# talmolab/track-mjx

Hardware: AMD Instinct MI355X
Metric: env-steps/sec (whole node), rodent task @ 4096 envs/GPU (higher is better)
Workload: dtype f32

## Files before the change

include/tmjx.h:

```cpp
#ifndef TMJX_H
#define TMJX_H
#include <stddef.h>
#include <stdint.h>

#ifdef __cplusplus
extern "C" {
#endif

#define TMJX_OK 0
#define TMJX_EINVAL (-22)
#define TMJX_ENOMEM (-12)
#define TMJX_EHIP (-5)

typedef struct tmjx_model tmjx_model;

typedef struct tmjx_layout_t {
  int32_t nq, nv, nu, nbody, ncon, nefc, obs_size, ref_obs_size, n_metrics, window;
  int32_t qpos, qvel, act, qacc_warmstart, time;
  int32_t xpos, xmat_torso, qfrc_actuator;
  int32_t prev_ctrl, action_buffer, done, steps_f;
  int32_t first_phys, first_obs, first_prev_ctrl;
  int32_t state_rows;
  int32_t i_clip_idx, i_start_frame, i_buffer_index, i_nan_count, istate_rows;
  int32_t ws_rows;
} tmjx_layout_t;

int tmjx_model_create(const void *blob, size_t nbytes, tmjx_model **out);
void tmjx_model_destroy(tmjx_model *m);
int tmjx_layout(const tmjx_model *m, tmjx_layout_t *out);

int tmjx_set_wrappers(tmjx_model *m, int episode_length, int auto_reset);
int tmjx_set_action_repeat(tmjx_model *m, int action_repeat);

int tmjx_clips_upload(tmjx_model *m, const float *position, const float *quaternion, const float *joints,
                      const float *body_positions, const float *angular_velocity, int n_clips, int n_frames);

int tmjx_reset(tmjx_model *m, float *state, int32_t *istate, const int32_t *clip_idx, const int32_t *start_frame,
               const float *qpos_noise, const float *qvel_noise, float *obs, float *workspace, int n_env, void *stream);

int tmjx_step(tmjx_model *m, float *state, int32_t *istate, const float *action, float *obs, float *reward,
              float *done, float *truncation, float *metrics, float *workspace, int n_env, void *stream);

int tmjx_physics_step(tmjx_model *m, float *state, const float *action, float *workspace, int n_env, void *stream);

int tmjx_physics(tmjx_model *m, float *state, const float *action, int n_substeps, float *workspace, int n_env,
                 void *stream);
int tmjx_forward(tmjx_model *m, float *state, float *workspace, int n_env, void *stream);

int tmjx_reward_obs(tmjx_model *m, float *state, int32_t *istate, const float *action, float *obs, float *reward,
                    float *done, float *truncation, float *metrics, float *workspace, int n_env, void *stream);

int tmjx_reward_frame(tmjx_model *m, float *state, int32_t *istate, const float *action, const float *frame_pos,
                      const float *frame_quat, const float *frame_joints, const float *frame_bodypos, const float *frame_angvel,
                      float *obs, float *reward, float *done, float *truncation, float *metrics, int n_env, void *stream);

int tmjx_gae(const float *truncation, const float *termination, const float *rewards, const float *values,
             const float *bootstrap, float lambda_, float discount, float *vs, float *advantages, int T, int B,
             void *stream);

typedef struct {
  int32_t T, B, A, Z;
  float reward_scaling, discounting, gae_lambda, clip_eps, entropy_cost, kl_weight;
  int32_t normalize_advantage;
  int32_t accumulate;
} tmjx_ppo_cfg_t;
int tmjx_ppo_scratch_floats(int T, int B);
int tmjx_ppo_loss(const tmjx_ppo_cfg_t *cfg, const float *logits, const float *raw_action, const float *behaviour_logp,
                  const float *noise, const float *baseline, const float *bootstrap, const float *reward, const float *discount,
                  const float *truncation, const float *fc2, float *dlogits, float *dbaseline, float *dfc2, float *scratch,
                  float *out, void *stream);

#define TMJX_PPO_PHASE_A 1
#define TMJX_PPO_PHASE_B 2
#define TMJX_PPO_PHASE_C 4
#define TMJX_PPO_PHASE_D 8
int tmjx_ppo_loss_phases(const tmjx_ppo_cfg_t *cfg, const float *logits, const float *raw_action, const float *behaviour_logp,
                         const float *noise, const float *baseline, const float *bootstrap, const float *reward, const float *discount,
                         const float *truncation, const float *fc2, float *dlogits, float *dbaseline, float *dfc2, float *scratch,
                         float *out, int phases, void *stream);

int tmjx_silu_ln_partial_floats(int rows, int H);
int tmjx_silu_ln_fwd(const float *z, const float *bias, const float *gamma, const float *beta, float *y, float *stats, int rows, int H,
                     float eps, void *stream);
int tmjx_silu_ln_bwd(const float *dy, const float *z, const float *bias, const float *gamma, const float *stats, float *dz, float *grads,
                     float *partial, int rows, int H, void *stream);
int tmjx_silu_ln_fwd_bf16(const float *z, const float *bias, const float *gamma, const float *beta, uint16_t *y16, int ldy16, float *stats, int rows, int H,
                          float eps, void *stream);
int tmjx_silu_ln_bwd_bf16(const float *dy, const float *z, const float *bias, const float *gamma, const float *stats, uint16_t *dz16, int lddz16, float *grads,
                          float *partial, int rows, int H, void *stream);

int tmjx_gather_normalize(const float *src, const int64_t *idx, const float *mean, const float *std, float *out, int T, int R, int B,
                          int W, void *stream);
int tmjx_gather_minibatch(const float *obs, const float *next_last, const float *raw_action, const float *log_prob, const float *reward, const float *discount,
                          const float *truncation, const int64_t *idx, const float *mean, const float *std, float *obs_n, float *next_n, float *raw_action_g,
                          float *scalars_g, int T, int R, int B, int W, int A, void *stream);
#define TMJX_MINIBATCH_STATE_WORDS (16 + 16 * 64)
typedef struct tmjx_minibatch_t {
  const float *obs, *next_last, *raw_action, *log_prob, *reward, *discount, *truncation;
  const int64_t *perm;
  const float *mean, *std;
  float *obs_n, *next_n, *raw_action_g, *scalars_g;
  float *eps, *noise;
  int64_t *state;
  uint64_t seed;
  int32_t T, R, B, W, A, Z, advance;
} tmjx_minibatch_t;
int tmjx_minibatch_begin(const tmjx_minibatch_t *mb, void *stream);
int tmjx_minibatch_begin_bf16(const tmjx_minibatch_t *mb, uint16_t *obs_n16, int ld16, void *stream);
int tmjx_philox4x32_10(const uint32_t *ctr_key_dev, uint32_t *out_dev, void *stream);

int tmjx_latent_concat_bwd(const float *dx, const float *eps, const float *fc2, float *dfc2, int n, int Z, int dx_stride, void *stream);
int tmjx_latent_concat_bwd_add(const float *dx, const float *eps, const float *fc2, const float *add, float *dfc2, int n, int Z, int dx_stride,
                               void *stream);

int tmjx_latent_concat(const float *fc2, const float *eps, const float *obs, float *x, int n, int Z, int obs_w, int ref_w,
                       int64_t obs_s0, int64_t obs_s1, const float *mean, const float *std, int x_stride, uint64_t seed, const int64_t *rng_state,
                       void *stream);
int tmjx_sample_action(const float *logits, const float *noise, float *raw, float *action_t, float *logp, int n, int A, uint64_t seed,
                       int64_t *rng_state, void *stream);

int tmjx_linear_act_ok(const float *A, int64_t lda, const float *W, int ldw, int K);
int tmjx_linear_act(const float *A, int64_t lda, const float *W, int ldw, const float *bias, float *C, int M, int N, int K,
                    const float *mean, const float *inv_std, void *stream);
int tmjx_linear_nolds(const float *A, int64_t sa_row, int64_t sa_k, const float *W, const float *bias, float *C, int M, int N, int K,
                      void *stream);
int tmjx_linear_nolds_norm(const float *A, int64_t sa_row, int64_t sa_k, const float *W, const float *bias, float *C, int M, int N, int K,
                           const float *mean, const float *inv_std, void *stream);

int tmjx_linear_nolds_bf16(const float *A, int64_t sa_row, int64_t sa_k, const uint16_t *W, int ldw, const float *bias, float *C, int M, int N, int K,
                           const float *mean, const float *inv_std, void *stream);

int tmjx_colsum_scratch_floats(int width);
int tmjx_colsum(const float *src, float *out, float *scratch, int rows, int width, void *stream);

typedef struct tmjx_colsum_problem_t { const float *partial; float *out; int32_t rows, width; } tmjx_colsum_problem_t;
int tmjx_colsum_grouped(const tmjx_colsum_problem_t *problems, int n, void *stream);

int tmjx_adam_clip(float *param, const float *grad, float *exp_avg, float *exp_avg_sq, const float *grad_norm, long long n, float lr,
                   float beta1, float beta2, float eps, float bias_correction1, float bias_correction2, float max_norm, void *stream);
int tmjx_adam_norm_floats(void);
int tmjx_adam_clip_norm(float *param, const float *grad, float *exp_avg, float *exp_avg_sq, float *norm_scratch, float *norm_out, long long n, float lr,
                        float beta1, float beta2, float eps, float bias_correction1, float bias_correction2, float max_norm, void *stream);

int tmjx_gemm_nt(const float *A, int lda, const float *W, int ldw, const float *bias, float *C, int ldc, int M, int N, int K, void *stream);
int tmjx_gemm_nn(const float *A, int lda, const float *W, int ldw, float *C, int ldc, int M, int N, int K, void *stream);
int tmjx_gemm_nt_silu_ln_ok(const float *A, int lda, const float *W, int ldw, int N);
int tmjx_gemm_nt_silu_ln(const float *A, int lda, const float *W, int ldw, const float *bias, const float *gamma, const float *beta, float *Z, float *Y,
                         int ldc, float *stats, int M, int N, int K, float eps, void *stream);
int tmjx_gemm_nn_ln_bwd_ok(const float *dY, int ldy, const float *W, int ldw, int N);
long long tmjx_gemm_nn_ln_bwd_partial_floats(int M, int N);
int tmjx_gemm_nn_ln_bwd(const float *dY, int ldy, const float *W, int ldw, const float *z, const float *bias, const float *gamma, const float *stats,
                        float *dz, float *partial, int M, int N, int K, void *stream);
int tmjx_gemm_nt_silu_ok(const float *A, int lda, const float *W, int ldw);
int tmjx_gemm_nt_silu(const float *A, int lda, const float *W, int ldw, const float *bias, float *Z, float *Y, int ldc, int M, int N, int K, void *stream);
int tmjx_silu_fwd(const float *z, const float *bias, float *y, long long rows, int N, void *stream);
int tmjx_silu_bwd(const float *dy, const float *z, const float *bias, float *dz, long long rows, int N, void *stream);
int tmjx_gemm_nn_silu_bwd_ok(const float *dY, int ldy, const float *W, int ldw);
int tmjx_gemm_nn_silu_bwd(const float *dY, int ldy, const float *W, int ldw, const float *z, const float *bias, float *dZ, int M, int N, int K, void *stream);
int tmjx_silu_bwd_rank1(const float *dy1, const float *w1, const float *z, const float *bias, float *dz, long long rows, int N, void *stream);
long long tmjx_head_dw_scratch_floats(int M, int K);
int tmjx_head_dw(const float *dy1, const float *x, int ldx, float *dw, float *db, float *scratch, int M, int K, void *stream);
#define TMJX_CHAIN_MAX_HIDDEN 4
typedef struct { const float *W, *bias, *gamma, *beta; float *z, *y, *stats; int32_t K, ldw; } tmjx_chain_layer_t;
typedef struct {
  const float *A; int32_t lda, M, n_hidden, epi;
  tmjx_chain_layer_t hidden[TMJX_CHAIN_MAX_HIDDEN];
  const float *Wf, *bf; float *outf; int32_t Nf, ldwf, ldof;
  float eps;
  int32_t rows_alloc;
  const float *lat_eps; float *lat_out; const float *prop; int32_t lat_Z, lat_ld, prop_w, prop_ld;
  void *prof;
} tmjx_chain_fwd_t;
int tmjx_chain_rows(int M);
int tmjx_chain_fwd_ok(const tmjx_chain_fwd_t *chain);
int tmjx_chain_fwd(const tmjx_chain_fwd_t *chain, void *stream);
typedef struct { const float *W; int32_t ldw; const float *z, *bias, *gamma, *stats; float *dz, *partial; } tmjx_chain_bwd_stage_t;
typedef struct {
  const float *G; int32_t ldg, Kg, M, n_stages, epi;
  tmjx_chain_bwd_stage_t stage[TMJX_CHAIN_MAX_HIDDEN];
  const float *W0; int32_t ldw0, dx_cols; float *dx; int32_t lddx;
  int32_t rows_alloc;
  void *prof;
} tmjx_chain_bwd_t;
int tmjx_chain_bwd_ok(const tmjx_chain_bwd_t *chain);
int tmjx_chain_bwd(const tmjx_chain_bwd_t *chain, void *stream);

int tmjx_head_fwd_ok(const float *x, int ldx, const float *w, int K);
int tmjx_head_fwd(const float *x, int ldx, const float *w, const float *bias, float *y, int M, int K, void *stream);
long long tmjx_gemm_dw_scratch_floats(int M, int N, int K);
int tmjx_gemm_dw(const float *dY, int ldy, const float *X, int ldx, float *dW, float *db, float *scratch, int M, int N, int K, void *stream);
typedef struct tmjx_dw_problem_t {
  const float *dY, *X;
  float *dW, *db, *scratch;
  int32_t ldy, ldx, lddw, M, N, K;
} tmjx_dw_problem_t;
int tmjx_gemm_dw_grouped(const tmjx_dw_problem_t *problems, int n, void *stream);
int tmjx_gemm_dw_grouped_wgs(const tmjx_dw_problem_t *probs, int n, int target_wgs, void *stream);

typedef struct tmjx_bf16_shadow_t {
  const float *src;
  uint16_t *dst, *dst_t;
  int32_t N, K, ld_src, ld_dst, ld_dst_t;
} tmjx_bf16_shadow_t;
int tmjx_bf16_shadow(const tmjx_bf16_shadow_t *items, int n, void *stream);
int tmjx_bgemm_nt(const void *A, int a_is_f32, int lda, const uint16_t *B, int ldb, const float *bias, float *C, int ldc, int M, int N, int K,
                  void *stream);
int tmjx_bgemm_row_tile_ok(int N);
int tmjx_bf16_z_bytes(void);
long long tmjx_bgemm_partial_floats(int M, int N, int sums);
int tmjx_bgemm_ln_fwd(const void *A, int a_is_f32, int lda, const uint16_t *B, int ldb, const float *bias, const float *gamma, const float *beta, uint16_t *Z16, int ldz,
                      uint16_t *Y16, int ldy16, float *stats, int M, int N, int K, float eps, void *stream);
int tmjx_bgemm_ln_bwd(const void *dY, int dy_is_f32, int ldy, const uint16_t *Bt, int ldb, const uint16_t *z16, int ldz, const float *bias, const float *gamma,
                      const float *stats, uint16_t *dZ16, int lddz, float *partial, int M, int N, int K, void *stream);
int tmjx_bgemm_silu_fwd(const void *A, int a_is_f32, int lda, const uint16_t *B, int ldb, const float *bias, uint16_t *Z16, int ldz, uint16_t *Y16, int ldy16,
                        float *Yf, int ldyf, int M, int N, int K, void *stream);
int tmjx_bgemm_silu_bwd(const void *dY, int dy_is_f32, int ldy, const uint16_t *Bt, int ldb, const uint16_t *z16, int ldz, const float *bias, uint16_t *dZ16, int lddz,
                        float *partial, int M, int N, int K, void *stream);
int tmjx_bf_silu_bwd(const float *dY, int ldy, const uint16_t *z16, int ldz, const float *bias, uint16_t *dZ16, int lddz, float *partial, int M, int N, void *stream);
int tmjx_bf_silu_bwd_rank1(const float *dy1, const float *w1, const uint16_t *z16, int ldz, const float *bias, uint16_t *dZ16, int lddz, float *partial, int M, int N,
                           void *stream);
long long tmjx_bgemm_dw_scratch_floats(int M, int N, int K);
int tmjx_bgemm_dw(const void *dY, int y_is_f32, int ldy, const void *X, int x_is_f32, int ldx, float *dW, int lddw, float *db, float *scratch,
                  int M, int N, int K, void *stream);
typedef struct tmjx_bdw_problem_t {
  const void *dY, *X;
  float *dW, *db, *scratch;
  int32_t y_is_f32, x_is_f32, ldy, ldx, lddw, M, N, K;
} tmjx_bdw_problem_t;
int tmjx_bgemm_dw_grouped(const tmjx_bdw_problem_t *problems, int n, int target_wgs, void *stream);

typedef struct tmjx_rollout_store_t {
  const float *obs; float *obs_dst0, *obs_dst1;
  const float *raw; float *raw_dst;
  const float *logp; float *logp_dst;
  const float *reward; float *reward_dst;
  const float *done; float *discount_dst;
  const float *trunc; float *trunc_dst;
  int32_t n, W, A;
  float *obs_dst2;
} tmjx_rollout_store_t;
int tmjx_rollout_store(const tmjx_rollout_store_t *s, void *stream);
int tmjx_clips_share(tmjx_model *m, const tmjx_model *owner);

int tmjx_stats_scratch_floats(int W);
int tmjx_stats_sums(const float *src, const float *mean, float *sums, float *scratch, long long rows, int W, void *stream);
int tmjx_stats_apply(const float *sums, float n_added, float *count, float *mean, float *summed_variance, float *std, int W, float std_min,
                     float std_max, void *stream);

int tmjx_debug_rows(const tmjx_model *m, const char *name, int *row0, int *count);

const char *tmjx_last_error(void);
const char *tmjx_version(void);

#ifdef __cplusplus
}
#endif
#endif
```

track_mjx_amd/agent/networks.py:

```python
from __future__ import annotations

import math
import os
from typing import Sequence

import torch
import torch.nn as nn
import torch.nn.functional as F


def _lecun_uniform_(w: torch.Tensor) -> None:
    fan_in = w.shape[1]
    lim = math.sqrt(3.0 / fan_in)
    with torch.no_grad():
        w.uniform_(-lim, lim)


def _lecun_normal_(w: torch.Tensor) -> None:
    fan_in = w.shape[1]
    std = math.sqrt(1.0 / fan_in) / 0.87962566103423978
    with torch.no_grad():
        nn.init.trunc_normal_(w, mean=0.0, std=std, a=-2 * std, b=2 * std)


class gemm_inputs:
    dtype = None
    shadows = None
    twins = None

    def __init__(self, dtype, shadows=None, twins=None):
        self.new = (dtype, shadows if dtype is not None else None, twins if dtype is not None else None)

    def __enter__(self):
        self.old = (gemm_inputs.dtype, gemm_inputs.shadows, gemm_inputs.twins)
        gemm_inputs.dtype, gemm_inputs.shadows, gemm_inputs.twins = self.new

    def __exit__(self, *a):
        gemm_inputs.dtype, gemm_inputs.shadows, gemm_inputs.twins = self.old
        return False

    @staticmethod
    def twin_of(x2: torch.Tensor, K: int):
        tw = gemm_inputs.twins
        if not tw or x2.dtype != torch.float32:
            return None
        hit = tw.get(x2.data_ptr())
        if hit is None:
            return None
        t16, width = hit
        Ke = _ceil64(K)
        if t16.shape[0] != x2.shape[0] or x2.stride(0) != width or K > width or Ke > t16.shape[1] or os.environ.get("TMJX_NO_BF16_TWIN"):
            return None
        return t16[:, :Ke]


def _hip_gemm_ok(*ts) -> bool:
    return gemm_inputs.dtype is None and all(t.is_cuda and t.dtype == torch.float32 for t in ts)


def _rows2d(x: torch.Tensor) -> torch.Tensor:
    x2 = x.reshape(-1, x.shape[-1])
    return x2 if x2.stride(1) == 1 and (x2.shape[0] == 1 or x2.stride(0) >= x2.shape[1]) else x2.contiguous()


def _launch(fn_name: str, dev, *args):
    import ctypes as C
    from .. import hip as _hip
    L = _hip.lib()
    with torch.cuda.device(dev):
        _hip.check(getattr(L, fn_name)(*args, C.c_void_p(torch.cuda.current_stream(dev).cuda_stream)), fn_name)


def _p(t):
    import ctypes as C
    return C.c_void_p(t.data_ptr()) if t is not None else None


def gemm_nt(x: torch.Tensor, w: torch.Tensor, bias: torch.Tensor | None = None) -> torch.Tensor:
    x = _rows2d(x)
    w = w if w.stride(1) == 1 else w.contiguous()
    M, K = x.shape
    N = w.shape[0]
    y = torch.empty((M, N), dtype=torch.float32, device=x.device)
    if N == 1 and _head_kernels() and K % 4 == 0 and x.data_ptr() % 16 == 0 and x.stride(0) % 4 == 0 and w.data_ptr() % 16 == 0:
        _launch("tmjx_head_fwd", x.device, _p(x), x.stride(0), _p(w), _p(bias), _p(y), M, K)
        return y
    _launch("tmjx_gemm_nt", x.device, _p(x), x.stride(0), _p(w), w.stride(0), _p(bias), _p(y), N, M, N, K)
    return y


def _head_kernels() -> bool:
    return os.environ.get("TMJX_HEAD_KERNELS", "1") != "0"


def gemm_nn(dy: torch.Tensor, w: torch.Tensor, cols: int | None = None) -> torch.Tensor:
    dy = _rows2d(dy)
    w = w if w.stride(1) == 1 else w.contiguous()
    M, N = dy.shape
    K = w.shape[1]
    dx = torch.empty((M, K), dtype=torch.float32, device=dy.device)
    _launch("tmjx_gemm_nn", dy.device, _p(dy), dy.stride(0), _p(w), w.stride(0), _p(dx), K, M, K if cols is None else int(cols), N)
    return dx


def gemm_dw(dy: torch.Tensor, x: torch.Tensor, with_bias: bool):
    from .. import hip as _hip
    dy, x = _rows2d(dy), _rows2d(x)
    M, N = dy.shape
    K = x.shape[1]
    dw = torch.empty((N, K), dtype=torch.float32, device=dy.device)
    db = torch.empty(N, dtype=torch.float32, device=dy.device) if with_bias else None
    if N == 1 and _head_kernels() and dy.stride(0) == 1:
        scratch = torch.empty(int(_hip.lib().tmjx_head_dw_scratch_floats(M, K)), dtype=torch.float32, device=dy.device)
        _launch("tmjx_head_dw", dy.device, _p(dy), _p(x), x.stride(0), _p(dw), _p(db), _p(scratch), M, K)
        return dw, db
    scratch = torch.empty(int(_hip.lib().tmjx_gemm_dw_scratch_floats(M, N, K)), dtype=torch.float32, device=dy.device)
    _launch("tmjx_gemm_dw", dy.device, _p(dy), dy.stride(0), _p(x), x.stride(0), _p(dw), _p(db), _p(scratch), M, N, K)
    return dw, db


def _ceil64(n: int) -> int:
    return (int(n) + 63) // 64 * 64


def _ld(x2: torch.Tensor) -> int:
    return x2.stride(0) if x2.shape[0] > 1 else (x2.shape[1] + 7) // 8 * 8


def bgemm_nt(x: torch.Tensor, wb: torch.Tensor, N: int, K: int, bias: torch.Tensor | None = None, out: torch.Tensor | None = None) -> torch.Tensor:
    x = _rows2d(x)
    M = x.shape[0]
    y = torch.empty((M, N), dtype=torch.float32, device=x.device) if out is None else out
    _launch("tmjx_bgemm_nt", x.device, _p(x), int(x.dtype == torch.float32), _ld(x), _p(wb), wb.stride(0), _p(bias), _p(y), max(y.stride(0), N), M, N, K)
    return y


def bgemm_dw(dy: torch.Tensor, x: torch.Tensor, with_bias: bool, out: torch.Tensor | None = None, out_bias: torch.Tensor | None = None):
    from .. import hip as _hip
    dy, x = _rows2d(dy), _rows2d(x)
    M, N = dy.shape
    K = x.shape[1]
    dw = torch.empty((N, K), dtype=torch.float32, device=dy.device) if out is None else out
    db = (torch.empty(N, dtype=torch.float32, device=dy.device) if out_bias is None else out_bias) if with_bias else None
    d = deferred_weight_grads.active
    if d is not None and d.group_bf16 and N > 1 and out is not None:
        d.bproblems.append((dy, x, dw, db))
        return dw, db
    scratch = torch.empty(int(_hip.lib().tmjx_bgemm_dw_scratch_floats(M, N, K)), dtype=torch.float32, device=dy.device)
    _launch("tmjx_bgemm_dw", dy.device, _p(dy), int(dy.dtype == torch.float32), _ld(dy), _p(x), int(x.dtype == torch.float32), _ld(x),
            _p(dw), dw.stride(0) if N > 1 else max(dw.stride(0), K), _p(db), _p(scratch), M, N, K)
    return dw, db


def bf16_z_dtype() -> torch.dtype:
    from .. import hip as _hip
    return torch.float32 if int(_hip.lib().tmjx_bf16_z_bytes()) == 4 else torch.bfloat16


def bgemm_ln_fwd(x, wb, N: int, K: int, bias, gamma, beta, eps: float):
    x = _rows2d(x)
    M = x.shape[0]
    z = torch.empty((M, N), dtype=bf16_z_dtype(), device=x.device)
    y = torch.empty((M, N), dtype=torch.bfloat16, device=x.device)
    stats = torch.empty((M, 2), dtype=torch.float32, device=x.device)
    _launch("tmjx_bgemm_ln_fwd", x.device, _p(x), int(x.dtype == torch.float32), _ld(x), _p(wb), wb.stride(0), _p(bias), _p(gamma), _p(beta), _p(z), N, _p(y), N,
            _p(stats), M, N, K, float(eps))
    return z, y, stats


def bgemm_ln_bwd(dy, wtb, N: int, K: int, z, bias, gamma, stats):
    from .. import hip as _hip
    dy = _rows2d(dy)
    M = dy.shape[0]
    dz = torch.empty((M, N), dtype=torch.bfloat16, device=dy.device)
    partial = torch.empty(int(_hip.lib().tmjx_bgemm_partial_floats(M, N, 3)), dtype=torch.float32, device=dy.device)
    _launch("tmjx_bgemm_ln_bwd", dy.device, _p(dy), int(dy.dtype == torch.float32), _ld(dy), _p(wtb), wtb.stride(0), _p(z), z.stride(0), _p(bias), _p(gamma), _p(stats),
            _p(dz), N, _p(partial), M, N, K)
    return dz, partial.view(-1, 3, N)


def bgemm_silu_fwd(x, wb, N: int, K: int, bias, y_f32: bool = False):
    x = _rows2d(x)
    M = x.shape[0]
    ld = (N + 7) // 8 * 8
    z = torch.empty((M, ld), dtype=bf16_z_dtype(), device=x.device)[:, :N]
    y = torch.empty((M, ld), dtype=torch.float32 if y_f32 else torch.bfloat16, device=x.device)
    _launch("tmjx_bgemm_silu_fwd", x.device, _p(x), int(x.dtype == torch.float32), _ld(x), _p(wb), wb.stride(0), _p(bias), _p(z), ld,
            None if y_f32 else _p(y), ld, _p(y) if y_f32 else None, ld, M, N, K)
    return z, y[:, :N]


def bgemm_silu_bwd(dy, wtb, N: int, K: int, z, bias):
    from .. import hip as _hip
    dy = _rows2d(dy)
    M = dy.shape[0]
    ld = (N + 7) // 8 * 8
    dz = torch.empty((M, ld), dtype=torch.bfloat16, device=dy.device)
    partial = torch.empty(int(_hip.lib().tmjx_bgemm_partial_floats(M, N, 1)), dtype=torch.float32, device=dy.device)
    _launch("tmjx_bgemm_silu_bwd", dy.device, _p(dy), int(dy.dtype == torch.float32), _ld(dy), _p(wtb), wtb.stride(0), _p(z), z.stride(0), _p(bias), _p(dz), ld,
            _p(partial), M, N, K)
    return dz[:, :N], partial.view(-1, N)


class Bf16Shadows:

    def __init__(self, linears, need_t=None):
        from .. import hip as _hip
        self.lins = list(linears)
        need_t = set(self.lins if need_t is None else need_t)
        dev = self.lins[0].weight.device
        self.w, self.wt = {}, {}
        items = []
        for lin in self.lins:
            N, K = lin.weight.shape
            self.w[lin] = torch.zeros((N, _ceil64(K)), dtype=torch.bfloat16, device=dev)
            if lin in need_t:
                self.wt[lin] = torch.zeros((K, _ceil64(N)), dtype=torch.bfloat16, device=dev)
            t = self.wt.get(lin)
            items.append(_hip.Bf16Shadow(lin.weight.data_ptr(), self.w[lin].data_ptr(), t.data_ptr() if t is not None else None, N, K, lin.weight.stride(0),
                                         self.w[lin].stride(0), t.stride(0) if t is not None else 0))
        self._chunks = [(_hip.Bf16Shadow * len(items[i:i + 24]))(*items[i:i + 24]) for i in range(0, len(items), 24)]
        self._ptrs = [lin.weight.data_ptr() for lin in self.lins]

    def refresh(self) -> None:
        if self._ptrs != [lin.weight.data_ptr() for lin in self.lins]:
            raise RuntimeError("a parameter moved after its bf16 shadow was built (build the shadows after the flat optimiser re-seats the parameters)")
        dev = self.lins[0].weight.device
        for arr in self._chunks:
            _launch("tmjx_bf16_shadow", dev, arr, len(arr))


def _bf16_ok(x, lin) -> bool:
    sh = gemm_inputs.shadows
    return (gemm_inputs.dtype == torch.bfloat16 and sh is not None and lin in sh.w and x.is_cuda and x.dtype == torch.float32
            and lin.out_features % 4 == 0)


def _colsum(dy: torch.Tensor) -> torch.Tensor:
    if not (dy.is_cuda and dy.dtype == torch.float32 and dy.dim() == 2 and dy.is_contiguous() and dy.shape[0] >= 1024):
        return dy.sum(0)
    import ctypes as C
    from .. import hip as _hip
    L = _hip.lib()
    rows, width = dy.shape
    out = torch.empty(width, dtype=torch.float32, device=dy.device)
    scratch = torch.empty(L.tmjx_colsum_scratch_floats(width), dtype=torch.float32, device=dy.device)
    with torch.cuda.device(dy.device):
        _hip.check(L.tmjx_colsum(C.c_void_p(dy.data_ptr()), C.c_void_p(out.data_ptr()), C.c_void_p(scratch.data_ptr()), rows, width,
                                 C.c_void_p(torch.cuda.current_stream(dy.device).cuda_stream)), "tmjx_colsum")
    return out


class deferred_weight_grads:
    active = None

    def __enter__(self):
        self.problems, self.keep, self.colsums = [], [], []
        self.bproblems, self.group_bf16 = [], os.environ.get("TMJX_BDW_GROUPED", "1") != "0"
        self.seen: set = set()
        deferred_weight_grads.active = self
        return self

    def __exit__(self, *a):
        deferred_weight_grads.active = None
        return False

    @staticmethod
    def _aligned(t):
        return t.data_ptr() % 16 == 0 and t.stride(0) % 4 == 0 and t.stride(1) == 1

    def try_add(self, dy2, x2, w, b):
        gw, gb = w.grad, (b.grad if b is not None else None)
        if gw is None or (b is not None and gb is None) or len(self.problems) >= 16:
            return None
        if not (self._aligned(dy2) and self._aligned(x2) and gw.stride(1) == 1 and gw.shape == w.shape):
            return None
        if id(w) in self.seen:
            mine = [q for q in self.problems if q[2].data_ptr() == gw.data_ptr()]
            self.problems = [q for q in self.problems if q[2].data_ptr() != gw.data_ptr()]
            self._launch_problems(mine)
            return None
        self.seen.add(id(w))
        self.problems.append((dy2, x2, gw, gb))
        return gw, gb

    def launch_subset(self, pick, target_wgs: int = 0):
        mine = [q for q in self.problems if pick(q[2])]
        self.problems = [q for q in self.problems if not pick(q[2])]
        self._launch_problems(mine, target_wgs)

    def launch(self):
        import ctypes as C
        from .. import hip as _hip
        L = _hip.lib()
        if self.colsums:
            dev = self.colsums[0][0].device
            arr = (_hip.ColsumProblem * len(self.colsums))(*[_hip.ColsumProblem(pt.data_ptr(), g.data_ptr(), nb, wd) for pt, g, nb, wd in self.colsums])
            with torch.cuda.device(dev):
                _hip.check(L.tmjx_colsum_grouped(arr, len(self.colsums), C.c_void_p(torch.cuda.current_stream(dev).cuda_stream)), "tmjx_colsum_grouped")
            self.keep += [t for c in self.colsums for t in c[:2]]
            self.colsums = []
        self._launch_problems(self.problems)
        self.problems = []
        self._launch_bproblems()

    def _launch_bproblems(self):
        import ctypes as C
        from .. import hip as _hip
        probs, self.bproblems = self.bproblems, []
        if not probs:
            return
        L = _hip.lib()
        dev = probs[0][0].device
        for at in range(0, len(probs), 24):
            grp = probs[at:at + 24]
            sizes = [int(L.tmjx_bgemm_dw_scratch_floats(dy.shape[0], dy.shape[1], x.shape[1])) for dy, x, _, _ in grp]
            scratch = torch.empty(sum((n + 3) // 4 * 4 for n in sizes), dtype=torch.float32, device=dev)
            arr = (_hip.BdwProblem * len(grp))()
            off = 0
            for i, (dy, x, dw, db) in enumerate(grp):
                N, K = dy.shape[1], x.shape[1]
                arr[i] = _hip.BdwProblem(dy.data_ptr(), x.data_ptr(), dw.data_ptr(), db.data_ptr() if db is not None else None, scratch.data_ptr() + 4 * off,
                                         int(dy.dtype == torch.float32), int(x.dtype == torch.float32), _ld(dy), _ld(x), dw.stride(0) if N > 1 else max(dw.stride(0), K),
                                         dy.shape[0], N, K)
                off += (sizes[i] + 3) // 4 * 4
            with torch.cuda.device(dev):
                _hip.check(L.tmjx_bgemm_dw_grouped(arr, len(grp), 0, C.c_void_p(torch.cuda.current_stream(dev).cuda_stream)), "tmjx_bgemm_dw_grouped")
            self.keep += [scratch] + [t for q in grp for t in q[:2]]

    def _launch_problems(self, problems, target_wgs: int = 0):
        import ctypes as C
        from .. import hip as _hip
        if not problems:
            return
        L = _hip.lib()
        dev = problems[0][0].device
        sizes = [int(L.tmjx_gemm_dw_scratch_floats(dy.shape[0], dy.shape[1], x.shape[1])) for dy, x, _, _ in problems]
        scratch = torch.empty(sum((n + 3) // 4 * 4 for n in sizes), dtype=torch.float32, device=dev)
        arr = (_hip.DwProblem * len(problems))()
        off = 0
        for i, (dy, x, gw, gb) in enumerate(problems):
            arr[i] = _hip.DwProblem(dy.data_ptr(), x.data_ptr(), gw.data_ptr(), gb.data_ptr() if gb is not None else None,
                                    scratch.data_ptr() + 4 * off, dy.stride(0), x.stride(0), gw.stride(0), dy.shape[0], dy.shape[1], x.shape[1])
            off += (sizes[i] + 3) // 4 * 4
        with torch.cuda.device(dev):
            _hip.check(L.tmjx_gemm_dw_grouped_wgs(arr, len(problems), int(target_wgs), C.c_void_p(torch.cuda.current_stream(dev).cuda_stream)), "tmjx_gemm_dw_grouped")
        self.keep += [scratch] + [t for q in problems for t in q[:2]]


def chain_fwd_desc(x2, hidden, final=None, kind="ln", eps=1e-6, out=None, latent=None):
    from .. import hip as _hip
    M, dev = x2.shape[0], x2.device
    d = _hip.ChainFwd()
    d.A, d.lda, d.M, d.n_hidden, d.epi, d.eps = x2.data_ptr(), x2.stride(0), M, len(hidden), 1 if kind == "ln" else 3, float(eps)
    saved = []
    d.rows_alloc = rows = int(_hip.lib().tmjx_chain_rows(M))
    for l, h in enumerate(hidden):
        w, b = h[0], h[1]
        z = torch.empty((M, 256), dtype=torch.float32, device=dev)
        y = torch.empty((rows, 256), dtype=torch.float32, device=dev)[:M]
        st = torch.empty((M, 2), dtype=torch.float32, device=dev) if kind == "ln" else None
        L = d.hidden[l]
        L.W, L.bias, L.z, L.y, L.K, L.ldw = w.data_ptr(), b.data_ptr(), z.data_ptr(), y.data_ptr(), w.shape[1], w.stride(0)
        if kind == "ln":
            L.gamma, L.beta, L.stats = h[2].data_ptr(), h[3].data_ptr(), st.data_ptr()
        saved.append((z, y, st))
    if final is not None:
        wf, bf = final
        Nf = wf.shape[0]
        if out is None:
            out = torch.empty((M,) if Nf == 1 else (M, Nf), dtype=torch.float32, device=dev)
        d.Wf, d.bf, d.outf, d.Nf, d.ldwf, d.ldof = wf.data_ptr(), (bf.data_ptr() if bf is not None else None), out.data_ptr(), Nf, wf.stride(0), (1 if Nf == 1 else out.stride(0))
    if latent is not None:
        leps, dec_in, prop = latent
        d.lat_eps, d.lat_out, d.prop = leps.data_ptr(), dec_in.data_ptr(), prop.data_ptr()
        d.lat_Z, d.lat_ld, d.prop_w, d.prop_ld = leps.shape[1], dec_in.stride(0), prop.shape[1], prop.stride(0)
    return d, saved, out


def chain_fwd(x2, hidden, final=None, kind="ln", eps=1e-6, latent=None):
    import ctypes as C
    d, saved, out = chain_fwd_desc(x2, hidden, final, kind, eps, latent=latent)
    _launch("tmjx_chain_fwd", x2.device, C.byref(d))
    return saved, out


def chain_fwd_ok(x2, hidden, final=None, kind="ln") -> bool:
    import ctypes as C
    from .. import hip as _hip
    if os.environ.get("TMJX_NO_CHAIN") or not (x2.is_cuda and x2.dtype == torch.float32 and x2.dim() == 2 and x2.stride(1) == 1):
        return False
    if any(h[0].shape[0] != 256 for h in hidden) or not (1 <= len(hidden) <= 4):
        return False
    return bool(_hip.lib().tmjx_chain_fwd_ok(C.byref(chain_fwd_desc(x2[:1], hidden, final, kind)[0])))


def chain_bwd(g, final_w, blocks, kind="ln", w0=None, dx_cols=None, prof=None, dx_ld=None):
    import ctypes as C
    from .. import hip as _hip
    L = _hip.lib()
    M, dev = g.shape[0], g.device
    d = _hip.ChainBwd()
    head = g.dim() == 1
    d.G, d.ldg, d.Kg, d.M, d.n_stages, d.epi = g.data_ptr(), (1 if head else g.stride(0)), (1 if head else g.shape[1]), M, len(blocks), 2 if kind == "ln" else 4
    dzs, partials = [], []
    nfl = int(L.tmjx_gemm_nn_ln_bwd_partial_floats(M, 256)) if kind == "ln" else 0
    d.rows_alloc = rows = int(L.tmjx_chain_rows(M))
    for i, blk in enumerate(blocks):
        S = d.stage[i]
        w = final_w if i == 0 else blocks[i - 1][0]
        S.W, S.ldw = w.data_ptr(), (w.stride(0) if w.dim() == 2 and w.shape[0] > 1 else 256)
        dz = torch.empty((rows, 256), dtype=torch.float32, device=dev)[:M]
        S.z, S.bias, S.dz = blk[1].data_ptr(), blk[2].data_ptr(), dz.data_ptr()
        if kind == "ln":
            pt = torch.empty(nfl, dtype=torch.float32, device=dev)
            S.gamma, S.stats, S.partial = blk[3].data_ptr(), blk[4].data_ptr(), pt.data_ptr()
            partials.append(pt)
        dzs.append(dz)
    dx = None
    if w0 is not None:
        cols = int(dx_cols)
        dx = torch.empty((M, (cols + 3) // 4 * 4 if dx_ld is None else int(dx_ld)), dtype=torch.float32, device=dev)
        d.W0, d.ldw0, d.dx_cols, d.dx, d.lddx = w0.data_ptr(), w0.stride(0), cols, dx.data_ptr(), dx.stride(0)
    if prof is not None:
        d.prof = prof.data_ptr()
    _launch("tmjx_chain_bwd", dev, C.byref(d))
    return dzs, (partials if kind == "ln" else None), dx


class _Layer:
    __slots__ = ("kind", "lin", "norm", "fused")

    def __init__(self, kind, lin, norm=None):
        from .. import hip as _hip
        self.kind, self.lin, self.norm = kind, lin, norm
        self.fused = kind == "silu" or (kind == "ln" and bool(_hip.lib().tmjx_bgemm_row_tile_ok(lin.out_features)))

    def params(self):
        return [self.lin.weight, self.lin.bias] + ([self.norm.weight, self.norm.bias] if self.kind == "ln" else [])


class _BfChainFn(torch.autograd.Function):

    @staticmethod
    def forward(ctx, x, layers, sh, dx_cols, last_y_f32, *params):
        import ctypes as C
        from .. import hip as _hip
        x2 = _rows2d(x)
        q = 4 if x2.dtype == torch.float32 else 8
        if x2.data_ptr() % 16 or x2.stride(0) % q or x2.stride(1) != 1:
            padded = torch.empty((x2.shape[0], (x2.shape[1] + q - 1) // q * q), dtype=x2.dtype, device=x2.device)
            padded[:, :x2.shape[1]].copy_(x2)
            x2 = padded[:, :x2.shape[1]]
        saved, h = [], x2
        t16 = gemm_inputs.twin_of(x2, layers[0].lin.weight.shape[1])
        for i, L in enumerate(layers):
            lin = L.lin
            N, K = lin.weight.shape
            last = i == len(layers) - 1 or layers[i + 1].kind == "head"
            hx = h
            if i == 0 and t16 is not None:
                h, hx, K = t16, t16[:, :K], t16.shape[1]
            if L.kind == "dense":
                y = bgemm_nt(h, sh.w[lin], N, K, lin.bias)
                saved.append((hx, None, None))
            elif L.kind == "head":
                y = gemm_nt(h, lin.weight, lin.bias)
                saved.append((h, None, None))
            elif L.kind == "silu":
                z, y = bgemm_silu_fwd(h, sh.w[lin], N, K, lin.bias, y_f32=last and last_y_f32)
                saved.append((hx, z, None))
            elif L.fused:
                z, y, stats = bgemm_ln_fwd(h, sh.w[lin], N, K, lin.bias, L.norm.weight, L.norm.bias, L.norm.eps)
                saved.append((hx, z, stats))
            else:
                z = bgemm_nt(h, sh.w[lin], N, K)
                stats = torch.empty((z.shape[0], 2), dtype=torch.float32, device=z.device)
                if last:
                    y = torch.empty_like(z)
                    _launch("tmjx_silu_ln_fwd", z.device, _p(z), _p(lin.bias), _p(L.norm.weight), _p(L.norm.bias), _p(y), _p(stats), z.shape[0], N, float(L.norm.eps))
                else:
                    y = torch.empty((z.shape[0], N), dtype=torch.bfloat16, device=z.device)
                    _launch("tmjx_silu_ln_fwd_bf16", z.device, _p(z), _p(lin.bias), _p(L.norm.weight), _p(L.norm.bias), _p(y), N, _p(stats), z.shape[0], N, float(L.norm.eps))
                saved.append((hx, z, stats))
            h = y
        ctx.layers, ctx.sh, ctx.dx_cols, ctx.saved, ctx.x_shape = layers, sh, dx_cols, saved, x.shape
        return h.view(*x.shape[:-1], h.shape[-1])

    @staticmethod
    def backward(ctx, dout):
        from .. import hip as _hip
        layers, sh, saved = ctx.layers, ctx.sh, ctx.saved
        Lh = _hip.lib()
        d = deferred_weight_grads.active
        g = _rows2d(dout)
        if g.data_ptr() % 16 or g.stride(0) % 4:
            g = g.contiguous()
        M = g.shape[0]
        g_is_dz = layers[-1].kind in ("dense", "head")
        grads = {}
        colsums = []

        def dest(p):
            if d is not None and p.grad is not None and p.grad.shape == p.shape and p.grad.stride(-1) == 1 and id(p) not in d.seen:
                d.seen.add(id(p))
                return p.grad
            return None

        def block_sums(L, partial):
            N = L.lin.out_features
            if L.kind == "ln":
                out = torch.empty((3, N), dtype=torch.float32, device=partial.device)
                colsums.append((partial, out, partial.shape[0], 3 * N))
                grads[id(L.norm.weight)], grads[id(L.norm.bias)], grads[id(L.lin.bias)] = out[0], out[1], out[2]
            else:
                out = torch.empty(N, dtype=torch.float32, device=partial.device)
                colsums.append((partial, out, partial.shape[0], N))
                grads[id(L.lin.bias)] = out

        dx = None
        for i in range(len(layers) - 1, -1, -1):
            L = layers[i]
            lin = L.lin
            N, K = lin.weight.shape
            h, z, stats = saved[i]
            if not g_is_dz:
                if L.kind == "ln":
                    gy = g if g.dtype == torch.float32 and g.is_contiguous() else g.float().contiguous()
                    dz = torch.empty((M, N), dtype=torch.bfloat16, device=z.device)
                    g3 = torch.empty((3, N), dtype=torch.float32, device=z.device)
                    partial = torch.empty(int(Lh.tmjx_silu_ln_partial_floats(M, N)), dtype=torch.float32, device=z.device)
                    z = z if z.dtype == torch.float32 else z.float()
                    _launch("tmjx_silu_ln_bwd_bf16", z.device, _p(gy), _p(z), _p(lin.bias), _p(L.norm.weight), _p(stats), _p(dz), N, _p(g3), _p(partial), M, N)
                    grads[id(L.norm.weight)], grads[id(L.norm.bias)], grads[id(lin.bias)] = g3[0], g3[1], g3[2]
                    g = dz
                else:
                    gy = g if g.dtype == torch.float32 else g.float()
                    ld = (N + 7) // 8 * 8
                    dz = torch.empty((M, ld), dtype=torch.bfloat16, device=z.device)
                    partial = torch.empty(int(Lh.tmjx_bgemm_partial_floats(M, N, 1)), dtype=torch.float32, device=z.device)
                    _launch("tmjx_bf_silu_bwd", z.device, _p(gy), gy.stride(0), _p(z), z.stride(0), _p(lin.bias), _p(dz), ld, _p(partial), M, N)
                    block_sums(L, partial.view(-1, N))
                    g = dz[:, :N]
            with_bias = L.kind in ("dense", "head")
            if L.kind == "head":
                dw, db = gemm_dw(g, h, True)
            else:
                dw, db = bgemm_dw(g, h, with_bias, out=dest(lin.weight), out_bias=dest(lin.bias) if with_bias else None)
            grads[id(lin.weight)] = dw
            if with_bias:
                grads[id(lin.bias)] = db
            if i > 0:
                P = layers[i - 1]
                Np = P.lin.out_features
                ph, pz, pstats = saved[i - 1]
                if L.kind == "head":
                    ld = (Np + 7) // 8 * 8
                    dzp = torch.empty((M, ld), dtype=torch.bfloat16, device=g.device)
                    partial = torch.empty(int(Lh.tmjx_bgemm_partial_floats(M, Np, 1)), dtype=torch.float32, device=g.device)
                    g1 = g.reshape(-1)
                    _launch("tmjx_bf_silu_bwd_rank1", g.device, _p(g1 if g1.is_contiguous() else g1.contiguous()), _p(lin.weight), _p(pz), pz.stride(0), _p(P.lin.bias), _p(dzp), ld,
                            _p(partial), M, Np)
                    block_sums(P, partial.view(-1, Np))
                    g, g_is_dz = dzp[:, :Np], True
                elif P.fused and P.kind == "ln":
                    g, partial = bgemm_ln_bwd(g, sh.wt[lin], Np, N, pz, P.lin.bias, P.norm.weight, pstats)
                    block_sums(P, partial)
                    g_is_dz = True
                elif P.fused:
                    g, partial = bgemm_silu_bwd(g, sh.wt[lin], Np, N, pz, P.lin.bias)
                    block_sums(P, partial)
                    g_is_dz = True
                else:
                    g = bgemm_nt(g, sh.wt[lin], Np, N)
                    g_is_dz = False
            elif ctx.needs_input_grad[0]:
                cols = K if ctx.dx_cols is None else int(ctx.dx_cols)
                dx = torch.empty((M, K), dtype=torch.float32, device=g.device)
                bgemm_nt(g, sh.wt[lin], cols, N, out=dx)
                dx = dx.view(ctx.x_shape)
        if colsums:
            arr = (_hip.ColsumProblem * len(colsums))(*[_hip.ColsumProblem(pt.data_ptr(), o.data_ptr(), nb, wd) for pt, o, nb, wd in colsums])
            _launch("tmjx_colsum_grouped", colsums[0][0].device, arr, len(colsums))
            ctx._keep = colsums
        out = []
        for L in layers:
            out += [grads.get(id(p)) for p in L.params()]
        return (dx, None, None, None, None, *out)


def bf16_chain(x, layers, dx_cols=None, last_y_f32=False):
    params = [p for L in layers for p in L.params()]
    return _BfChainFn.apply(x, layers, gemm_inputs.shadows, dx_cols, last_y_f32, *params)


def _bf16_chain_ok(x) -> bool:
    sh = gemm_inputs.shadows
    return gemm_inputs.dtype == torch.bfloat16 and sh is not None and x.is_cuda and x.dtype in (torch.float32, torch.bfloat16) and not os.environ.get("TMJX_NO_BF16_CHAIN")



class _F32ChainFn(torch.autograd.Function):

    @staticmethod
    def forward(ctx, x, layers, dx_cols, latent, *params):
        x2 = _rows2d(x)
        hid, last = layers[:-1], layers[-1]
        kind = hid[0].kind
        hidden = [(L.lin.weight, L.lin.bias, L.norm.weight, L.norm.bias) if kind == "ln" else (L.lin.weight, L.lin.bias) for L in hid]
        eps = float(hid[0].norm.eps) if kind == "ln" else 0.0
        dec_in = None
        if latent is not None:
            leps, prop = latent
            wd = leps.shape[1] + prop.shape[1]
            dec_in = torch.empty((x2.shape[0], (wd + 3) // 4 * 4), dtype=torch.float32, device=x2.device)
            latent = (leps, dec_in, prop)
        saved, out = chain_fwd(x2, hidden, (last.lin.weight, last.lin.bias), kind, eps, latent=latent)
        flat = [t for z, y, st in saved for t in ((z, y, st) if kind == "ln" else (z, y))]
        ctx.save_for_backward(x2, *flat, *params)
        ctx.layers, ctx.dx_cols, ctx.x_shape, ctx.kind, ctx.nflat = layers, dx_cols, x.shape, kind, len(flat)
        res = out.view(*x.shape[:-1], last.lin.out_features) if last.kind == "dense" else out.view(*x.shape[:-1], 1)
        if dec_in is None:
            return res
        xd = dec_in[:, :wd]
        ctx.mark_non_differentiable(xd)
        return res, xd

    @staticmethod
    def backward(ctx, dout, *_unused):
        from .. import hip as _hip
        layers, kind = ctx.layers, ctx.kind
        hid, last = layers[:-1], layers[-1]
        st_ = ctx.saved_tensors
        x2, flat, params = st_[0], st_[1:1 + ctx.nflat], st_[1 + ctx.nflat:]
        per = 3 if kind == "ln" else 2
        saved = [flat[per * i:per * i + per] for i in range(len(hid))]
        pit = iter(params)
        P = [[next(pit) for _ in L.params()] for L in layers]
        Lh = _hip.lib()
        dev = dout.device
        M = x2.shape[0]
        d = deferred_weight_grads.active
        grads: dict = {}
        wf, bf = P[-1][0], P[-1][1]
        y_last = saved[-1][1]
        if last.kind == "head":
            g = dout.reshape(-1)
            g = g if g.is_contiguous() else g.contiguous()
            K = wf.shape[1]
            dwh, dbh = torch.empty((1, K), dtype=torch.float32, device=dev), torch.empty(1, dtype=torch.float32, device=dev)
            scratch = torch.empty(int(Lh.tmjx_head_dw_scratch_floats(M, K)), dtype=torch.float32, device=dev)
            _launch("tmjx_head_dw", dev, _p(g), _p(y_last), y_last.stride(0), _p(dwh), _p(dbh), _p(scratch), M, K)
            grads[(len(layers) - 1, 0)], grads[(len(layers) - 1, 1)] = dwh, dbh
            ctx._keep = scratch
        else:
            g = _rows2d(dout)
            if g.data_ptr() % 16 or g.stride(0) % 4:
                g = g.contiguous()
            got = d.try_add(g, y_last, last.lin.weight, last.lin.bias) if d is not None else None
            dw, db = got if got is not None else gemm_dw(g, y_last, True)
            grads[(len(layers) - 1, 0)], grads[(len(layers) - 1, 1)] = dw, db
        if kind == "ln":
            blocks = [(P[l][0], saved[l][0], P[l][1], P[l][2], saved[l][2]) for l in range(len(hid) - 1, -1, -1)]
        else:
            blocks = [(P[l][0], saved[l][0], P[l][1]) for l in range(len(hid) - 1, -1, -1)]
        want_dx = ctx.needs_input_grad[0]
        cols = (x2.shape[1] if ctx.dx_cols is None else int(ctx.dx_cols)) if want_dx else None
        dzs, partials, dx = chain_bwd(g, wf, blocks, kind, P[0][0] if want_dx else None, cols, dx_ld=x2.shape[1] if want_dx else None)
        for i, dz in enumerate(dzs):
            l = len(hid) - 1 - i
            L = hid[l]
            xin = x2 if l == 0 else saved[l - 1][1]
            if kind == "ln":
                got = d.try_add(dz, xin, L.lin.weight, None) if d is not None else None
                grads[(l, 0)] = got[0] if got is not None else gemm_dw(dz, xin, False)[0]
                g3 = torch.empty((3, 256), dtype=torch.float32, device=dev)
                nblk = partials[i].numel() // 768
                if d is not None and len(d.colsums) < 16:
                    d.colsums.append((partials[i], g3, nblk, 768))
                else:
                    one = (_hip.ColsumProblem * 1)(_hip.ColsumProblem(partials[i].data_ptr(), g3.data_ptr(), nblk, 768))
                    _launch("tmjx_colsum_grouped", dev, one, 1)
                grads[(l, 2)], grads[(l, 3)], grads[(l, 1)] = g3[0], g3[1], g3[2]
            else:
                got = d.try_add(dz, xin, L.lin.weight, L.lin.bias) if d is not None else None
                grads[(l, 0)], grads[(l, 1)] = got if got is not None else gemm_dw(dz, xin, True)
        out = [grads.get((l, j)) for l, L in enumerate(layers) for j in range(len(L.params()))]
        return (dx.view(ctx.x_shape) if dx is not None else None, None, None, None, *out)


def f32_chain(x, layers, dx_cols=None, latent=None):
    params = [p for L in layers for p in L.params()]
    return _F32ChainFn.apply(x, layers, dx_cols, latent, *params)


def _f32_chain_ok(x, layers, dx_cols=None) -> bool:
    if gemm_inputs.dtype is not None or torch.is_autocast_enabled() or os.environ.get("TMJX_NO_CHAIN") or not (x.is_cuda and x.dtype == torch.float32):
        return False
    if x.requires_grad and torch.is_grad_enabled() and (x.shape[-1] if dx_cols is None else int(dx_cols)) > 128:
        return False
    hid, last = layers[:-1], layers[-1]
    if not hid or any(L.lin.out_features != 256 or L.lin.bias is None for L in hid) or last.lin.bias is None or last.lin.in_features != 256:
        return False
    kind = hid[0].kind
    hidden = [(L.lin.weight, L.lin.bias, L.norm.weight, L.norm.bias) if kind == "ln" else (L.lin.weight, L.lin.bias) for L in hid]
    return chain_fwd_ok(_rows2d(x), hidden, (last.lin.weight, last.lin.bias), kind)


class _BlockLink:
    __slots__ = ("y_ptr", "y_shape", "ctx", "dz_given", "grads")

    def __init__(self):
        self.y_ptr, self.y_shape, self.ctx, self.dz_given, self.grads = None, None, None, False, None


class ln_bwd_links:
    active = False
    last = None

    def __enter__(self):
        self._prev = (ln_bwd_links.active, ln_bwd_links.last)
        ln_bwd_links.active, ln_bwd_links.last = not os.environ.get("TMJX_NO_LN_BWD_FUSION"), None
        return self

    def __exit__(self, *a):
        ln_bwd_links.active, ln_bwd_links.last = self._prev
        return False

    @staticmethod
    def producer_of(x2):
        l = ln_bwd_links.last
        if ln_bwd_links.active and l is not None and l.y_ptr == x2.data_ptr() and l.y_shape == tuple(x2.shape) and x2.is_contiguous():
            return l
        return None


def _dx_through_block(dy2, w, link):
    import ctypes as C
    from .. import hip as _hip
    L = _hip.lib()
    x2, wp, z, b, gamma, stats = link.ctx.saved_tensors
    M, H = z.shape
    dz = torch.empty_like(z)
    nfl = int(L.tmjx_gemm_nn_ln_bwd_partial_floats(M, H))
    nblk = nfl // (3 * H)
    partial = torch.empty(nfl, dtype=torch.float32, device=z.device)
    grads = torch.empty((3, H), dtype=torch.float32, device=z.device)
    p = lambda t: C.c_void_p(t.data_ptr())
    with torch.cuda.device(z.device):
        stream = C.c_void_p(torch.cuda.current_stream(z.device).cuda_stream)
        _hip.check(L.tmjx_gemm_nn_ln_bwd(p(dy2), dy2.stride(0), p(w), w.stride(0), p(z), p(b), p(gamma), p(stats), p(dz), p(partial), M, H, dy2.shape[1], stream),
                   "tmjx_gemm_nn_ln_bwd")
        d = deferred_weight_grads.active
        if d is not None and len(d.colsums) < 16:
            d.colsums.append((partial, grads, nblk, 3 * H))
        else:
            one = (_hip.ColsumProblem * 1)(_hip.ColsumProblem(partial.data_ptr(), grads.data_ptr(), nblk, 3 * H))
            _hip.check(L.tmjx_colsum_grouped(one, 1, stream), "tmjx_colsum_grouped")
    link.dz_given, link.grads = True, grads
    return dz


def _fusable_dx(dy2, w, link, dx_cols) -> bool:
    if link is None or dx_cols is not None or link.ctx is None:
        return False
    import ctypes as C
    from .. import hip as _hip
    z = link.ctx.saved_tensors[2]
    return bool(z.shape[1] == w.shape[1] and _hip.lib().tmjx_gemm_nn_ln_bwd_ok(C.c_void_p(dy2.data_ptr()), dy2.stride(0), C.c_void_p(w.data_ptr()), w.stride(0), z.shape[1]))


class _HipDenseFn(torch.autograd.Function):

    @staticmethod
    def forward(ctx, x, w, b, dx_cols):
        x2 = _rows2d(x)
        ctx.save_for_backward(x2, w)
        ctx.has_bias, ctx.dx_cols, ctx.x_shape = b is not None, dx_cols, x.shape
        ctx.params = (w, b)
        ctx.producer = ln_bwd_links.producer_of(x2)
        ln_bwd_links.last = None
        return gemm_nt(x2, w, b).view(*x.shape[:-1], w.shape[0])

    @staticmethod
    def backward(ctx, dy):
        x2, w = ctx.saved_tensors
        dy2 = _rows2d(dy)
        if ctx.needs_input_grad[0] and _fusable_dx(dy2, w, ctx.producer, ctx.dx_cols):
            dx = _dx_through_block(dy2, w, ctx.producer).view(ctx.x_shape)
        else:
            dx = gemm_nn(dy2, w, ctx.dx_cols).view(ctx.x_shape) if ctx.needs_input_grad[0] else None
        d = deferred_weight_grads.active
        got = d.try_add(dy2, x2, *ctx.params) if d is not None else None
        dw, db = got if got is not None else gemm_dw(dy2, x2, ctx.has_bias)
        return dx, dw, db, None


class _HipSiluDenseFn(torch.autograd.Function):

    @staticmethod
    def forward(ctx, x, w, b):
        import ctypes as C
        from .. import hip as _hip
        x2 = _rows2d(x)
        M, K = x2.shape
        N = w.shape[0]
        z = torch.empty((M, N), dtype=torch.float32, device=x2.device)
        y = torch.empty_like(z)
        L = _hip.lib()
        if L.tmjx_gemm_nt_silu_ok(_p(x2), x2.stride(0), _p(w), w.stride(0)):
            _launch("tmjx_gemm_nt_silu", x2.device, _p(x2), x2.stride(0), _p(w), w.stride(0), _p(b), _p(z), _p(y), N, M, N, K)
        else:
            _launch("tmjx_gemm_nt", x2.device, _p(x2), x2.stride(0), _p(w), w.stride(0), None, _p(z), N, M, N, K)
            _launch("tmjx_silu_fwd", x2.device, _p(z), _p(b), _p(y), M, N)
        ctx.save_for_backward(x2, w, z, b)
        ctx.params, ctx.x_shape = (w, b), x.shape
        return y.view(*x.shape[:-1], N)

    @staticmethod
    def backward(ctx, dy):
        x2, w, z, b = ctx.saved_tensors
        M, N = z.shape
        dy2 = _rows2d(dy).contiguous()
        dz = torch.empty_like(z)
        _launch("tmjx_silu_bwd", z.device, _p(dy2), _p(z), _p(b), _p(dz), M, N)
        dx = gemm_nn(dz, w).view(ctx.x_shape) if ctx.needs_input_grad[0] else None
        d = deferred_weight_grads.active
        got = d.try_add(dz, x2, *ctx.params) if d is not None else None
        dw, db = got if got is not None else gemm_dw(dz, x2, True)
        return dx, dw, db


class _ValueChainFn(torch.autograd.Function):

    @staticmethod
    def forward(ctx, x, lins, *params):
        x2 = _rows2d(x)
        M = x2.shape[0]
        h, flat = x2, []
        for lin in lins[:-1]:
            N, K = lin.weight.shape
            z = torch.empty((M, N), dtype=torch.float32, device=x2.device)
            y = torch.empty_like(z)
            _launch("tmjx_gemm_nt_silu", x2.device, _p(h), h.stride(0), _p(lin.weight), lin.weight.stride(0), _p(lin.bias), _p(z), _p(y), N, M, N, K)
            flat += [h, z]
            h = y
        head = lins[-1]
        out = gemm_nt(h, head.weight, head.bias)
        ctx.save_for_backward(*flat, h, *params)
        ctx.lins, ctx.x_shape = lins, x.shape
        return out.view(*x.shape[:-1], 1)

    @staticmethod
    def backward(ctx, dout):
        from .. import hip as _hip
        lins = ctx.lins
        nl = len(lins)
        st = ctx.saved_tensors
        saved = [(st[2 * i], st[2 * i + 1]) for i in range(nl - 1)]
        h_last = st[2 * (nl - 1)]
        W = [(st[2 * (nl - 1) + 1 + 2 * i], st[2 * (nl - 1) + 2 + 2 * i]) for i in range(nl)]
        L = _hip.lib()
        dev = dout.device
        dy1 = dout.reshape(-1)
        dy1 = dy1 if dy1.is_contiguous() else dy1.contiguous()
        M = dy1.shape[0]
        head = lins[-1]
        grads = {}
        K = head.in_features
        dwh, dbh = torch.empty((1, K), dtype=torch.float32, device=dev), torch.empty(1, dtype=torch.float32, device=dev)
        scratch = torch.empty(int(L.tmjx_head_dw_scratch_floats(M, K)), dtype=torch.float32, device=dev)
        _launch("tmjx_head_dw", dev, _p(dy1), _p(h_last), h_last.stride(0), _p(dwh), _p(dbh), _p(scratch), M, K)
        grads[id(head.weight)], grads[id(head.bias)] = dwh, dbh
        last = lins[-2]
        dz = torch.empty_like(saved[-1][1])
        _launch("tmjx_silu_bwd_rank1", dev, _p(dy1), _p(W[-1][0]), _p(saved[-1][1]), _p(W[-2][1]), _p(dz), M, last.out_features)
        d = deferred_weight_grads.active
        dx = None
        for i in range(nl - 2, -1, -1):
            lin = lins[i]
            w_i = W[i][0]
            xin, _ = saved[i]
            got = d.try_add(dz, xin, lin.weight, lin.bias) if d is not None else None
            dw, db = got if got is not None else gemm_dw(dz, xin, True)
            grads[id(lin.weight)], grads[id(lin.bias)] = dw, db
            if i > 0:
                prev, pz = lins[i - 1], saved[i - 1][1]
                dzp = torch.empty_like(pz)
                _launch("tmjx_gemm_nn_silu_bwd", dev, _p(dz), dz.stride(0), _p(w_i), w_i.stride(0), _p(pz), _p(W[i - 1][1]), _p(dzp), M, prev.out_features, lin.out_features)
                dz = dzp
            elif ctx.needs_input_grad[0]:
                dx = gemm_nn(dz, w_i).view(ctx.x_shape)
        ctx._keep = scratch
        out = []
        for lin in lins:
            out += [grads[id(lin.weight)], grads[id(lin.bias)]]
        return (dx, None, *out)


def _value_chain_ok(x2, lins) -> bool:
    from .. import hip as _hip
    if os.environ.get("TMJX_VALUE_CHAIN", "1") == "0" or len(lins) < 2 or lins[-1].out_features != 1 or lins[-1].bias is None:
        return False
    L = _hip.lib()
    if x2.data_ptr() % 16 or x2.stride(0) % 4 or x2.stride(1) != 1:
        return False
    for lin in lins[:-1]:
        if lin.bias is None or lin.out_features % 4 or lin.in_features % 4 or lin.weight.data_ptr() % 16 or lin.weight.stride(0) % 4 or lin.bias.data_ptr() % 16:
            return False
    if not (lins[-1].in_features % 4 == 0 and lins[-1].weight.data_ptr() % 16 == 0 and bool(L.tmjx_gemm_nt_silu_ok(_p(x2), x2.stride(0), _p(lins[0].weight), lins[0].weight.stride(0)))):
        return False
    return all(bool(L.tmjx_gemm_nn_silu_bwd_ok(None, lin.out_features, _p(lin.weight), lin.weight.stride(0))) for lin in lins[1:-1])


class _BfDenseFn(torch.autograd.Function):

    @staticmethod
    def forward(ctx, x, w, b, lin, dx_cols):
        x2 = _rows2d(x)
        if x2.data_ptr() % 16 or x2.stride(0) % 4:
            x2 = x2.contiguous()
        sh = gemm_inputs.shadows
        ctx.save_for_backward(x2)
        ctx.lin, ctx.sh, ctx.params, ctx.dx_cols, ctx.x_shape = lin, sh, (w, b), dx_cols, x.shape
        N, K = w.shape
        return bgemm_nt(x2, sh.w[lin], N, K, b).view(*x.shape[:-1], N)

    @staticmethod
    def backward(ctx, dy):
        (x2,) = ctx.saved_tensors
        w, b = ctx.params
        N, K = w.shape
        dy2 = _rows2d(dy)
        if dy2.data_ptr() % 16 or dy2.stride(0) % 4:
            dy2 = dy2.contiguous()
        dx = None
        if ctx.needs_input_grad[0]:
            cols = K if ctx.dx_cols is None else int(ctx.dx_cols)
            dx = torch.empty((dy2.shape[0], K), dtype=torch.float32, device=dy2.device)
            bgemm_nt(dy2, ctx.sh.wt[ctx.lin], cols, N, out=dx)
            dx = dx.view(ctx.x_shape)
        d = deferred_weight_grads.active
        gw = w.grad if (d is not None and w.grad is not None and w.grad.shape == w.shape and w.grad.stride(1) == 1 and id(w) not in d.seen) else None
        gb = b.grad if (b is not None and gw is not None and b.grad is not None) else None
        if gw is not None:
            d.seen.add(id(w))
        dw, db = bgemm_dw(dy2, x2, b is not None, out=gw, out_bias=gb)
        return dx, dw, db, None, None


class _Dense(nn.Linear):
    def forward(self, x):
        rows = x.numel() // x.shape[-1]
        if _bf16_ok(x, self):
            if torch.is_grad_enabled() and (self.weight.requires_grad or x.requires_grad):
                return _BfDenseFn.apply(x, self.weight, self.bias, self, None)
            return bgemm_nt(x, gemm_inputs.shadows.w[self], self.out_features, self.in_features, self.bias).view(*x.shape[:-1], self.out_features)
        if x.is_cuda and x.dtype == torch.float32 and self.weight.dtype == torch.float32:
            if torch.is_grad_enabled() and (self.weight.requires_grad or x.requires_grad):
                return _HipDenseFn.apply(x, self.weight, self.bias, None)
            return gemm_nt(x, self.weight, self.bias).view(*x.shape[:-1], self.out_features)
        return F.linear(x, self.weight, self.bias)


def _dense(i: int, o: int, init=_lecun_uniform_) -> nn.Linear:
    lin = _Dense(i, o)
    init(lin.weight)
    nn.init.zeros_(lin.bias)
    return lin


class _SiluLayerNormFn(torch.autograd.Function):

    @staticmethod
    def forward(ctx, z, bias, gamma, beta, eps):
        import ctypes as C
        from .. import hip as _hip
        H = z.shape[-1]
        rows = z.numel() // H
        z = z.contiguous()
        y = torch.empty_like(z)
        stats = torch.empty((rows, 2), dtype=torch.float32, device=z.device)
        L = _hip.lib()
        with torch.cuda.device(z.device):
            stream = C.c_void_p(torch.cuda.current_stream(z.device).cuda_stream)
            _hip.check(L.tmjx_silu_ln_fwd(*[C.c_void_p(t.data_ptr()) for t in (z, bias, gamma, beta, y, stats)], rows, H, float(eps), stream),
                       "tmjx_silu_ln_fwd")
        ctx.save_for_backward(z, bias, gamma, stats)
        return y

    @staticmethod
    def backward(ctx, dy):
        import ctypes as C
        from .. import hip as _hip
        z, bias, gamma, stats = ctx.saved_tensors
        H = z.shape[-1]
        rows = z.numel() // H
        dy = dy.contiguous()
        dz = torch.empty_like(z)
        grads = torch.empty((3, H), dtype=torch.float32, device=z.device)
        L = _hip.lib()
        partial = torch.empty(L.tmjx_silu_ln_partial_floats(rows, H), dtype=torch.float32, device=z.device)
        with torch.cuda.device(z.device):
            stream = C.c_void_p(torch.cuda.current_stream(z.device).cuda_stream)
            _hip.check(L.tmjx_silu_ln_bwd(*[C.c_void_p(t.data_ptr()) for t in (dy, z, bias, gamma, stats, dz, grads, partial)], rows, H, stream),
                       "tmjx_silu_ln_bwd")
        return dz, grads[2], grads[0], grads[1], None


def _block_fusable(x2, w) -> bool:
    if not _hip_gemm_ok(x2, w) or os.environ.get("TMJX_NO_FUSED_BLOCK"):
        return False
    from .. import hip as _hip
    import ctypes as C
    return bool(_hip.lib().tmjx_gemm_nt_silu_ln_ok(C.c_void_p(x2.data_ptr()), x2.stride(0), C.c_void_p(w.data_ptr()), w.stride(0), w.shape[0]))


class _HipBlockFn(torch.autograd.Function):

    @staticmethod
    def forward(ctx, x2, w, b, gamma, beta, eps, dx_cols):
        import ctypes as C
        from .. import hip as _hip
        M, K = x2.shape
        N = w.shape[0]
        z = torch.empty((M, N), dtype=torch.float32, device=x2.device)
        y = torch.empty_like(z)
        stats = torch.empty((M, 2), dtype=torch.float32, device=x2.device)
        p = lambda t: C.c_void_p(t.data_ptr())
        with torch.cuda.device(x2.device):
            _hip.check(_hip.lib().tmjx_gemm_nt_silu_ln(p(x2), x2.stride(0), p(w), w.stride(0), p(b), p(gamma), p(beta), p(z), p(y), N, p(stats), M, N, K,
                                                       float(eps), C.c_void_p(torch.cuda.current_stream(x2.device).cuda_stream)), "tmjx_gemm_nt_silu_ln")
        ctx.save_for_backward(x2, w, z, b, gamma, stats)
        ctx.dx_cols, ctx.param = dx_cols, w
        ctx.producer = ln_bwd_links.producer_of(x2)
        ctx.link = None
        if ln_bwd_links.active:
            ctx.link = link = _BlockLink()
            link.y_ptr, link.y_shape, link.ctx = y.data_ptr(), tuple(y.shape), ctx
            ln_bwd_links.last = link
        return y

    @staticmethod
    def backward(ctx, dy):
        import ctypes as C
        from .. import hip as _hip
        x2, w, z, b, gamma, stats = ctx.saved_tensors
        M, N = z.shape
        dy = dy.contiguous()
        if ctx.link is not None:
            ctx.link.ctx = None
        if ctx.link is not None and ctx.link.dz_given:
            dz, grads = dy, ctx.link.grads
            ctx.link.dz_given, ctx.link.grads = False, None
        else:
            dz = torch.empty_like(z)
            grads = torch.empty((3, N), dtype=torch.float32, device=z.device)
            L = _hip.lib()
            partial = torch.empty(L.tmjx_silu_ln_partial_floats(M, N), dtype=torch.float32, device=z.device)
            with torch.cuda.device(z.device):
                _hip.check(L.tmjx_silu_ln_bwd(*[C.c_void_p(t.data_ptr()) for t in (dy, z, b, gamma, stats, dz, grads, partial)], M, N,
                                              C.c_void_p(torch.cuda.current_stream(z.device).cuda_stream)), "tmjx_silu_ln_bwd")
        if ctx.needs_input_grad[0] and _fusable_dx(dz, w, ctx.producer, ctx.dx_cols):
            dx = _dx_through_block(dz, w, ctx.producer)
        else:
            dx = gemm_nn(dz, w, ctx.dx_cols) if ctx.needs_input_grad[0] else None
        d = deferred_weight_grads.active
        got = d.try_add(dz, x2, ctx.param, None) if d is not None else None
        dw = got[0] if got is not None else gemm_dw(dz, x2, False)[0]
        return dx, dw, grads[2], grads[0], grads[1], None, None


class _Block(nn.Module):
    FUSED_WIDTHS = (64, 128, 256, 512, 1024)

    def __init__(self, i: int, o: int):
        super().__init__()
        self.dense = _dense(i, o)
        self.norm = nn.LayerNorm(o, eps=1e-6)
        self.dx_cols = None

    def forward(self, x):
        if x.is_cuda and x.dtype == torch.float32 and self.dense.out_features in self.FUSED_WIDTHS and not torch.is_autocast_enabled():
            x2 = _rows2d(x)
            if torch.is_grad_enabled() and _block_fusable(x2, self.dense.weight):
                y = _HipBlockFn.apply(x2, self.dense.weight, self.dense.bias, self.norm.weight, self.norm.bias, self.norm.eps, self.dx_cols)
                return y.view(*x.shape[:-1], self.dense.out_features)
            if _bf16_ok(x2, self.dense):
                if torch.is_grad_enabled():
                    z = _BfDenseFn.apply(x2, self.dense.weight, None, self.dense, self.dx_cols)
                else:
                    z = bgemm_nt(x2, gemm_inputs.shadows.w[self.dense], self.dense.out_features, self.dense.in_features)
            elif not torch.is_grad_enabled():
                z = gemm_nt(x2, self.dense.weight)
            else:
                z = _HipDenseFn.apply(x2, self.dense.weight, None, self.dx_cols)
            y = _SiluLayerNormFn.apply(z, self.dense.bias, self.norm.weight, self.norm.bias, self.norm.eps)
            return y.view(*x.shape[:-1], self.dense.out_features)
        return self.norm(F.silu(self.dense(x)))


class _LatentConcatFn(torch.autograd.Function):

    @staticmethod
    def forward(ctx, fc2, eps, obs, ref, handle=None):
        import ctypes as C
        from .. import hip as _hip
        ctx.handle = handle
        n, Z = eps.shape
        W = obs.shape[1]
        fc2, eps, obs = fc2.contiguous(), eps.contiguous(), obs.contiguous()
        wd = Z + W - ref
        x = torch.empty((n, (wd + 3) // 4 * 4), dtype=torch.float32, device=fc2.device)
        p = lambda t: C.c_void_p(t.data_ptr())
        with torch.cuda.device(fc2.device):
            _hip.check(_hip.lib().tmjx_latent_concat(p(fc2), p(eps), p(obs), p(x), n, Z, W, ref, obs.stride(0), obs.stride(1), None, None, x.shape[1], 0, None,
                                                     C.c_void_p(torch.cuda.current_stream(fc2.device).cuda_stream)), "tmjx_latent_concat")
        ctx.save_for_backward(fc2, eps)
        return x[:, :wd]

    @staticmethod
    def backward(ctx, dx):
        import ctypes as C
        from .. import hip as _hip
        fc2, eps = ctx.saved_tensors
        n, Z = eps.shape
        dx = dx.contiguous()
        dfc2 = torch.empty_like(fc2)
        p = lambda t: C.c_void_p(t.data_ptr())
        add = ctx.handle.take() if ctx.handle is not None else None
        if add is not None and (add.shape != fc2.shape or not add.is_contiguous()):
            raise RuntimeError("_LatentConcatFn: the pending fc2 gradient does not fit this forward pass")
        with torch.cuda.device(fc2.device):
            stream = C.c_void_p(torch.cuda.current_stream(fc2.device).cuda_stream)
            if add is None:
                _hip.check(_hip.lib().tmjx_latent_concat_bwd(p(dx), p(eps), p(fc2), p(dfc2), n, Z, dx.shape[1], stream), "tmjx_latent_concat_bwd")
            else:
                _hip.check(_hip.lib().tmjx_latent_concat_bwd_add(p(dx), p(eps), p(fc2), p(add), p(dfc2), n, Z, dx.shape[1], stream), "tmjx_latent_concat_bwd_add")
        return dfc2, None, None, None, None


class _LatentViewFn(torch.autograd.Function):

    @staticmethod
    def forward(ctx, fc2, eps, x, handle=None):
        ctx.handle = handle
        ctx.save_for_backward(fc2.contiguous(), eps.contiguous())
        return x.view_as(x)

    @staticmethod
    def backward(ctx, dx):
        return (_LatentConcatFn.backward(ctx, dx)[0], None, None, None)


class LatentGradHandle:

    def __init__(self, fc2: torch.Tensor):
        self.ptr, self.shape, self._g = fc2.data_ptr(), tuple(fc2.shape), None

    def matches(self, fc2: torch.Tensor) -> bool:
        return fc2.data_ptr() == self.ptr

    def add(self, g: torch.Tensor) -> None:
        if self._g is not None:
            raise RuntimeError("LatentGradHandle: a gradient is already parked on this forward pass")
        self._g = g

    def take(self):
        g, self._g = self._g, None
        return g

    @property
    def pending(self) -> bool:
        return self._g is not None


class IntentionPolicy(nn.Module):

    def __init__(self, obs_size: int, reference_obs_size: int, action_size: int, latents: int = 60,
                 encoder_layers: Sequence[int] = (1024, 1024), decoder_layers: Sequence[int] = (1024, 1024)):
        super().__init__()
        self.reference_obs_size, self.latents, self.action_size = reference_obs_size, latents, action_size
        enc, d = [], reference_obs_size
        for h in encoder_layers:
            enc.append(_Block(d, h)); d = h
        self.encoder = nn.Sequential(*enc)
        self.fc2 = _dense(d, 2 * latents, _lecun_normal_)
        dec, d = [], latents + (obs_size - reference_obs_size)
        for h in decoder_layers:
            dec.append(_Block(d, h)); d = h
        self.decoder = nn.Sequential(*dec)
        dec[0].dx_cols = latents
        self.head = _dense(d, 2 * action_size)

    def forward(self, obs: torch.Tensor, eps: torch.Tensor | None = None, deterministic: bool = False, return_fc2: bool = False):
        traj = obs[..., :self.reference_obs_size]
        prev, self.latent_grad_handle = getattr(self, "latent_grad_handle", None), None
        if prev is not None and prev.pending:
            raise RuntimeError("IntentionPolicy: the fc2 gradient parked on the previous forward pass (LatentGradHandle.add) was never consumed by a "
                               "backward pass through that forward — it would have been dropped")
        chains = _bf16_chain_ok(obs) and all(m.out_features % 4 == 0 for m in (self.fc2, self.head))
        if chains:
            if getattr(self, "_enc_chain", None) is None:
                self._enc_chain = [_Layer("ln", b.dense, b.norm) for b in self.encoder] + [_Layer("dense", self.fc2)]
                self._dec_chain = [_Layer("ln", b.dense, b.norm) for b in self.decoder] + [_Layer("dense", self.head)]
            fc2 = bf16_chain(traj, self._enc_chain)
        else:
            if getattr(self, "_enc_f32", None) is None and obs.is_cuda:
                self._enc_f32 = [_Layer("ln", b.dense, b.norm) for b in self.encoder] + [_Layer("dense", self.fc2)]
                self._dec_f32 = [_Layer("ln", b.dense, b.norm) for b in self.decoder] + [_Layer("dense", self.head)]
            xlat = None
            if obs.is_cuda and _f32_chain_ok(traj, self._enc_f32):
                obs2 = obs.reshape(-1, obs.shape[-1])
                if (not deterministic and obs.dtype == torch.float32 and obs2.shape[0] * 2 * self.latents >= 2 * self.latents * 1024 and self.latents % 4 == 0
                        and (obs.shape[-1] - self.reference_obs_size) % 2 == 0 and obs2.stride(1) == 1 and obs2.stride(0) % 2 == 0 and self.reference_obs_size % 2 == 0
                        and os.environ.get("TMJX_CHAIN_LATENT") == "1"):
                    if eps is None:
                        eps = torch.randn(obs.shape[:-1] + (self.latents,), dtype=torch.float32, device=obs.device)
                    eps2 = eps.reshape(-1, self.latents).contiguous()
                    fc2, xlat = f32_chain(traj, self._enc_f32, latent=(eps2, obs2[:, self.reference_obs_size:]))
                else:
                    fc2 = f32_chain(traj, self._enc_f32)
            else:
                with ln_bwd_links():
                    h = self.encoder(traj)
                    fc2 = self.fc2(h)
        mean, logvar = torch.chunk(fc2, 2, dim=-1)
        if (not deterministic and fc2.is_cuda and fc2.dtype == torch.float32 and obs.dtype == torch.float32 and not torch.is_autocast_enabled()
                and fc2.numel() >= 2 * self.latents * 1024):
            lead = fc2.shape[:-1]
            if eps is None:
                eps = torch.randn_like(mean)
            handle = LatentGradHandle(fc2.reshape(-1, fc2.shape[-1])) if (fc2.requires_grad and fc2.is_contiguous()) else None
            if not chains and xlat is not None:
                x = _LatentViewFn.apply(fc2.reshape(-1, fc2.shape[-1]), eps.reshape(-1, self.latents), xlat, handle)
            else:
                x = _LatentConcatFn.apply(fc2.reshape(-1, fc2.shape[-1]), eps.reshape(-1, self.latents), obs.reshape(-1, obs.shape[-1]), self.reference_obs_size, handle)
            self.latent_grad_handle = handle
            x = x.view(*lead, x.shape[-1])
            if chains:
                logits = bf16_chain(x, self._dec_chain, dx_cols=self.latents)
            elif _f32_chain_ok(x, self._dec_f32, self.latents):
                logits = f32_chain(x, self._dec_f32, dx_cols=self.latents)
            else:
                with ln_bwd_links():
                    logits = self.head(self.decoder(x))
            if return_fc2:
                return logits, fc2
            return logits, mean, logvar
        if deterministic:
            z = mean
        else:
            if eps is None:
                eps = torch.randn_like(mean)
            z = mean + eps * torch.exp(0.5 * logvar)
        x = torch.cat([z, obs[..., self.reference_obs_size:]], dim=-1)
        logits = bf16_chain(x, self._dec_chain) if chains else self.head(self.decoder(x))
        if return_fc2:
            return logits, fc2
        return logits, mean, logvar


class _NoCtx:
    def save_for_backward(self, *a):
        pass


class ValueNet(nn.Module):

    def __init__(self, obs_size: int, hidden: Sequence[int] = (1024, 1024)):
        super().__init__()
        layers, d = [], obs_size
        for h in hidden:
            layers += [_dense(d, h), nn.SiLU()]; d = h
        layers.append(_dense(d, 1))
        self.net = nn.Sequential(*layers)

    def forward(self, obs):
        if _bf16_chain_ok(obs) and len(self.net) > 1:
            if getattr(self, "_chain", None) is None:
                dense = [m for m in self.net if isinstance(m, nn.Linear)]
                self._chain = [_Layer("silu", m) for m in dense[:-1]]
                head = dense[-1]
                if head.out_features == 1 and head.in_features % 4 == 0 and head.in_features <= 1024 and not os.environ.get("TMJX_NO_CHAIN_HEAD"):
                    self._chain.append(_Layer("head", head))
            h = bf16_chain(obs, self._chain, last_y_f32=True)
            if self._chain[-1].kind == "head":
                return h.squeeze(-1)
            return self.net[-1](h).squeeze(-1)
        if obs.is_cuda and obs.dtype == torch.float32 and gemm_inputs.dtype is None:
            h = obs
            dense = [m for m in self.net if isinstance(m, nn.Linear)]
            if len(dense) > 1 and dense[-1].out_features == 1:
                if getattr(self, "_f32_chain", None) is None:
                    self._f32_chain = [_Layer("silu", m) for m in dense[:-1]] + [_Layer("head", dense[-1])]
                if os.environ.get("TMJX_VALUE_CHAIN", "1") != "0" and _f32_chain_ok(obs, self._f32_chain):
                    return f32_chain(obs, self._f32_chain).squeeze(-1)
            if torch.is_grad_enabled() and any(p.requires_grad for p in self.parameters()) and _value_chain_ok(_rows2d(obs), dense):
                return _ValueChainFn.apply(obs, dense, *[p for lin in dense for p in (lin.weight, lin.bias)]).squeeze(-1)
            for lin in dense[:-1]:
                if torch.is_grad_enabled() and (lin.weight.requires_grad or h.requires_grad):
                    h = _HipSiluDenseFn.apply(h, lin.weight, lin.bias)
                else:
                    h = _HipSiluDenseFn.forward(_NoCtx(), h, lin.weight, lin.bias)
            return dense[-1](h).squeeze(-1)
        return self.net(obs).squeeze(-1)


class NormalTanh:
    MIN_STD = 0.001
    LOG2 = math.log(2.0)

    @staticmethod
    def params(logits):
        loc, raw = torch.chunk(logits, 2, dim=-1)
        return loc, F.softplus(raw) + NormalTanh.MIN_STD

    @staticmethod
    def sample_no_postprocessing(logits, noise=None):
        loc, scale = NormalTanh.params(logits)
        if noise is None:
            noise = torch.randn_like(loc)
        return loc + scale * noise

    @staticmethod
    def _fldj(x):
        return 2.0 * (NormalTanh.LOG2 - x - F.softplus(-2.0 * x))

    @staticmethod
    def log_prob(logits, raw_action):
        loc, scale = NormalTanh.params(logits)
        lp = -0.5 * ((raw_action - loc) / scale) ** 2 - torch.log(scale) - 0.5 * math.log(2 * math.pi)
        return (lp - NormalTanh._fldj(raw_action)).sum(-1)

    @staticmethod
    def entropy(logits, noise=None):
        loc, scale = NormalTanh.params(logits)
        ent = 0.5 + 0.5 * math.log(2 * math.pi) + torch.log(scale)
        x = NormalTanh.sample_no_postprocessing(logits, noise)
        return (ent + NormalTanh._fldj(x)).sum(-1)

    @staticmethod
    def postprocess(raw_action):
        return torch.tanh(raw_action)

    @staticmethod
    def mode(logits):
        return torch.tanh(torch.chunk(logits, 2, dim=-1)[0])


class RunningStatistics:

    def __init__(self, size: int, device, std_min: float = 1e-6, std_max: float = 1e6):
        self.count = torch.zeros((), dtype=torch.float32, device=device)
        self.mean = torch.zeros(size, dtype=torch.float32, device=device)
        self.summed_variance = torch.zeros(size, dtype=torch.float32, device=device)
        self.std = torch.ones(size, dtype=torch.float32, device=device)
        self.std_min, self.std_max = std_min, std_max

    @torch.no_grad()
    def update(self, batch: torch.Tensor, group=None, distributed: bool | None = None) -> None:
        import torch.distributed as dist
        if distributed is None:
            distributed = dist.is_available() and dist.is_initialized() and dist.get_world_size(group) > 1
        flat = batch.reshape(-1, batch.shape[-1])
        if not flat.is_contiguous():
            flat = flat.contiguous()
        rows, W = flat.shape
        n_added = float(rows * (dist.get_world_size(group) if distributed else 1))
        if flat.is_cuda and flat.dtype == torch.float32 and W % 4 == 0:
            import ctypes as C
            from .. import hip as _hip
            L = _hip.lib()
            p = lambda t: C.c_void_p(t.data_ptr())
            if getattr(self, "_sums", None) is None:
                self._sums = torch.empty(2 * W, dtype=torch.float32, device=flat.device)
                self._scratch = torch.empty(L.tmjx_stats_scratch_floats(W), dtype=torch.float32, device=flat.device)
            with torch.cuda.device(flat.device):
                stream = C.c_void_p(torch.cuda.current_stream(flat.device).cuda_stream)
                _hip.check(L.tmjx_stats_sums(p(flat), p(self.mean), p(self._sums), p(self._scratch), rows, W, stream), "tmjx_stats_sums")
                if distributed:
                    dist.all_reduce(self._sums, group=group)
                _hip.check(L.tmjx_stats_apply(p(self._sums), n_added, p(self.count), p(self.mean), p(self.summed_variance), p(self.std), W,
                                              float(self.std_min), float(self.std_max), stream), "tmjx_stats_apply")
            return
        d = flat - self.mean
        sums = torch.cat([d.sum(0), (d * d).sum(0)])
        if distributed:
            dist.all_reduce(sums, group=group)
        count = self.count + n_added
        upd = sums[:W] / count
        self.summed_variance.add_(sums[W:] - upd * sums[:W])
        self.mean.add_(upd); self.count.copy_(count)
        self.std.copy_(torch.sqrt(torch.clamp(self.summed_variance, min=0) / count).clamp(self.std_min, self.std_max))

    def normalize(self, x: torch.Tensor) -> torch.Tensor:
        return (x - self.mean) / self.std

    def state_dict(self):
        return {"count": self.count, "mean": self.mean, "summed_variance": self.summed_variance, "std": self.std}
```

track_mjx_amd/csrc/mlp_chain.h:

```cpp
#pragma once
#define GEMM_ACT_ONLY
#include "gemm_kernels.h"

#define CH_NT 512
#define CH_WSTAGE (32 * 260)
template <int MT> struct ChainLds {
  static constexpr int BM = 16 * MT, YIMG = BM * 256, RED = 4 * BM * 8, TOTAL = YIMG + 2 * CH_WSTAGE + RED;
  static_assert(2 * (BM + 8) * GEMM_LDA <= YIMG, "the first layer's A stages live in the Y image region");
};

template <int MT, int NI, bool BT, bool A_LDS>
struct ChainGemm {
  static constexpr int BM = 16 * MT, BN = 128 * NI, A_ROWS = BM + 8;
  static constexpr int A_PASS = A_LDS ? 0 : (BM * 8 + CH_NT - 1) / CH_NT, B_PASS = BN / 64, NPASS = A_PASS + B_PASS;
  static constexpr int LDB_N = BN + 4, A_STAGE = A_ROWS * GEMM_LDA;
  static constexpr int NMFMA = 4 * MT * NI, NFR = MT + (BT ? NI : 4 * NI);
  static constexpr int SPREAD = (NMFMA - NFR) / (NPASS + 1) > 0 ? (NMFMA - NFR) / (NPASS + 1) : 1;
  struct Stage { gf4 v[NPASS]; int m[NPASS]; };
  struct Frag { gf4 a[MT], b[NI]; };
  static constexpr int T4 = A_LDS ? BM / 8 : 0, TRK = MT >= 4 ? 2 : 1;
  const float *A, *W;
  float *ast, *yimg, *wst, *tr_dst;
  int lda, ldw, M, N, K, m0, t, li, kq, nw;
  const float *pa[A_PASS > 0 ? A_PASS : 1], *pb[B_PASS];
  Stage R0, R1;
  Frag F0, F1;

  __device__ __forceinline__ void init(const float *A_, int lda_, int M_, int m0_, const float *W_, int ldw_, int N_, int K_, float *yimg_, float *wst_, float *tr_ = nullptr) {
    A = A_; lda = lda_; M = M_; m0 = m0_; W = W_; ldw = ldw_; N = N_; K = K_; yimg = yimg_; ast = yimg_; wst = wst_;
    tr_dst = tr_ ? tr_ + (long long)m0_ * 256 : nullptr;
    t = threadIdx.x; li = t & 15; kq = (t & 63) >> 4; nw = (t >> 6) * 16 * NI;
#pragma unroll
    for (int p = 0; p < A_PASS; p++) {
      const int f = t + CH_NT * p, r = f < BM * 8 ? f >> 3 : 0, c4 = f & 7;
      pa[p] = A + (long long)min(m0 + r, M - 1) * lda + 4 * c4;
    }
#pragma unroll
    for (int p = 0; p < B_PASS; p++) {
      const int f = t + CH_NT * p;
      if (BT) { const int r = f >> 3, c4 = f & 7; pb[p] = W + (long long)min(r, N - 1) * ldw + 4 * c4; }
      else { const int r = f / (BN / 4), c4 = f % (BN / 4); pb[p] = W + (long long)r * ldw + min(4 * c4, ((N + 3) & ~3) - 4); }
    }
  }
  __device__ __forceinline__ void gload(Stage &R, int k0) {
#pragma unroll
    for (int p = 0; p < A_PASS; p++) {
      const int f = t + CH_NT * p, r = f >> 3, c4 = f & 7;
      const bool ok = f < BM * 8 && m0 + r < M;
      R.v[p] = gemm_ld4<true>(A, (long long)(m0 + (ok ? r : 0)) * lda, k0 + 4 * c4, K, ok, R.m[p]);
    }
#pragma unroll
    for (int p = 0; p < B_PASS; p++) {
      const int f = t + CH_NT * p;
      if (BT) {
        const int r = f >> 3, c4 = f & 7;
        const bool ok = r < N;
        R.v[A_PASS + p] = gemm_ld4<true>(W, (long long)(ok ? r : 0) * ldw, k0 + 4 * c4, K, ok, R.m[A_PASS + p]);
      } else {
        const int r = f / (BN / 4), c4 = f % (BN / 4);
        const bool ok = k0 + r < K;
        R.v[A_PASS + p] = gemm_ld4<true>(W, (long long)(ok ? k0 + r : 0) * ldw, 4 * c4, N, ok, R.m[A_PASS + p]);
      }
    }
  }
  __device__ __forceinline__ float *b_slot(float *sb, int f) const {
    if (BT) { const int r = f >> 3, c4 = f & 7; return sb + r * 32 + ((c4 ^ ((r >> 1) & 7)) << 2); }
    const int r = f / (BN / 4), c4 = f % (BN / 4);
    return sb + r * LDB_N + 4 * c4;
  }
  template <bool MASKED>
  __device__ __forceinline__ void swrite(const Stage &R, int stage) {
    float *sa = ast + stage * A_STAGE, *sb = wst + stage * CH_WSTAGE;
#pragma unroll
    for (int p = 0; p < A_PASS; p++) {
      const int f = t + CH_NT * p, r = f < BM * 8 ? f >> 3 : BM + ((f >> 3) & 7), c4 = f & 7;
      *reinterpret_cast<gf4 *>(sa + r * GEMM_LDA + 4 * c4) = MASKED ? gemm_mask4(R.v[p], R.m[p]) : R.v[p];
    }
#pragma unroll
    for (int p = 0; p < B_PASS; p++)
      *reinterpret_cast<gf4 *>(b_slot(sb, t + CH_NT * p)) = MASKED ? gemm_mask4(R.v[A_PASS + p], R.m[A_PASS + p]) : R.v[A_PASS + p];
  }
  __device__ __forceinline__ void gload_fast(Stage &R, int k0) {
    const int k0c = k0 + GEMM_BK <= K ? k0 : 0;
#pragma unroll
    for (int p = 0; p < A_PASS; p++) R.v[p] = *reinterpret_cast<const gf4 *>(pa[p] + k0c);
#pragma unroll
    for (int p = 0; p < B_PASS; p++) R.v[A_PASS + p] = *reinterpret_cast<const gf4 *>(pb[p] + (BT ? (long long)k0c : (long long)k0c * ldw));
  }
  __device__ __forceinline__ void fread(Frag &F, int stage, int c, int kt) {
    const float *sb = wst + stage * CH_WSTAGE;
    if (A_LDS) {
#pragma unroll
      for (int a = 0; a < MT; a++) F.a[a] = *reinterpret_cast<const gf4 *>(yimg + (16 * a + li) * 256 + (((8 * kt + 4 * c + kq) ^ li) << 2));
    } else {
      const float *sa = ast + stage * A_STAGE;
#pragma unroll
      for (int a = 0; a < MT; a++) F.a[a] = *reinterpret_cast<const gf4 *>(sa + (16 * a + li) * GEMM_LDA + 16 * c + 4 * kq);
    }
    if (BT) {
#pragma unroll
      for (int b = 0; b < NI; b++) F.b[b] = *reinterpret_cast<const gf4 *>(sb + (nw + 16 * b + li) * 32 + (((4 * c + kq) ^ (li >> 1)) << 2));
    } else {
#pragma unroll
      for (int e = 0; e < 4; e++) {
        const float *q = sb + (16 * c + 4 * kq + e) * LDB_N + nw + NI * li;
        if constexpr (NI == 2) { const gf2 v = *reinterpret_cast<const gf2 *>(q); F.b[0][e] = v.x; F.b[1][e] = v.y; }
        else F.b[0][e] = q[0];
      }
    }
  }
  __device__ __forceinline__ void mma(const Frag &F, gf4 (&acc)[MT][NI]) {
#pragma unroll
    for (int e = 0; e < 4; e++)
#pragma unroll
      for (int a = 0; a < MT; a++)
#pragma unroll
        for (int b = 0; b < NI; b++) {
          if constexpr (BT || NI == 2) acc[a][b] = __builtin_amdgcn_mfma_f32_16x16x4f32(F.b[b][e], F.a[a][e], acc[a][b], 0, 0, 0);
          else acc[a][b] = __builtin_amdgcn_mfma_f32_16x16x4f32(F.a[a][e], F.b[b][e], acc[a][b], 0, 0, 0);
        }
  }
  template <bool FASTS, int TR = 0>
  __device__ __forceinline__ void kstep(gf4 (&acc)[MT][NI], Stage &RW, int stage, int kt) {
    gf4 trv[TR > 0 ? TR : 1];
    fread(F1, stage, 1, kt);
    swrite<!FASTS>(RW, stage ^ 1);
    mma(F0, acc);
#pragma unroll
    for (int i = 0; i < NFR; i++) { GEMM_SGB(SG_MFMA, 1, 0); GEMM_SGB(SG_DS_READ, 1, 0); }
#pragma unroll
    for (int i = 0; i < NPASS; i++) { GEMM_SGB(SG_MFMA, SPREAD, 0); if (!FASTS) GEMM_SGB(SG_VALU, 12, 0); GEMM_SGB(SG_DS_WRITE, 1, 0); }
    GEMM_SGB(SG_MFMA, NMFMA, 0);
    __syncthreads();
    fread(F0, stage ^ 1, 0, kt + 1);
    if constexpr (TR > 0) {
#pragma unroll
      for (int j = 0; j < TR; j++) {
        const int f = t + CH_NT * min(kt * TRK + j, T4 - 1), row = f >> 6, c4 = f & 63;
        trv[j] = *reinterpret_cast<const gf4 *>(yimg + row * 256 + ((c4 ^ (row & 15)) << 2));
      }
    }
    if (FASTS) gload_fast(RW, (kt + 3) * GEMM_BK); else gload(RW, (kt + 3) * GEMM_BK);
    mma(F1, acc);
    if constexpr (TR > 0) {
#pragma unroll
      for (int j = 0; j < TR; j++) {
        const int f = t + CH_NT * min(kt * TRK + j, T4 - 1);
        *reinterpret_cast<gf4 *>(tr_dst + (long long)(f >> 6) * 256 + 4 * (f & 63)) = trv[j];
      }
    }
#pragma unroll
    for (int i = 0; i < NFR + TR; i++) { GEMM_SGB(SG_MFMA, 1, 0); GEMM_SGB(SG_DS_READ, 1, 0); }
#pragma unroll
    for (int i = 0; i < NPASS; i++) { GEMM_SGB(SG_MFMA, SPREAD, 0); GEMM_SGB(SG_VALU, FASTS ? 2 : GEMM_LOAD_VALU, 0); GEMM_SGB(SG_VMEM_READ, 1, 0); }
#pragma unroll
    for (int i = 0; i < TR; i++) { GEMM_SGB(SG_MFMA, 1, 0); GEMM_SGB(SG_VALU, 4, 0); GEMM_SGB(SG_VMEM_WRITE, 1, 0); }
    GEMM_SGB(SG_MFMA, NMFMA, 0);
  }
  __device__ __forceinline__ void early() {
    if (A_LDS) { gload_fast(R0, 0); gload_fast(R1, GEMM_BK); } else { gload(R0, 0); gload(R1, GEMM_BK); }
  }
  __device__ __forceinline__ void late() {
    if (A_LDS) { swrite<false>(R0, 0); gload_fast(R0, 2 * GEMM_BK); } else { swrite<true>(R0, 0); gload(R0, 2 * GEMM_BK); }
    __syncthreads();
    fread(F0, 0, 0, 0);
  }
  __device__ __forceinline__ void loop(gf4 (&acc)[MT][NI]) {
    if constexpr (A_LDS) {
      constexpr int NTRS = 2 * (((T4 + TRK - 1) / TRK + 1) / 2);
      int kt = 0;
      for (; kt < NTRS; kt += 2) { kstep<true, TRK>(acc, R1, 0, kt); kstep<true, TRK>(acc, R0, 1, kt + 1); }
      for (; kt < 8; kt += 2) { kstep<true, 0>(acc, R1, 0, kt); kstep<true, 0>(acc, R0, 1, kt + 1); }
      return;
    }
    const int nk = (K + GEMM_BK - 1) / GEMM_BK;
    int kt = 0;
    const int nfast = (A_LDS || (K % GEMM_BK) == 0) ? nk : max(0, (nk - 4) & ~1);
    for (; kt + 1 < nfast; kt += 2) { kstep<true>(acc, R1, 0, kt); kstep<true>(acc, R0, 1, kt + 1); }
    if (kt < nfast) { kstep<true>(acc, R1, 0, kt); kt = nk; }
    if constexpr (!A_LDS) {
      for (; kt + 1 < nk; kt += 2) { kstep<false>(acc, R1, 0, kt); kstep<false>(acc, R0, 1, kt + 1); }
      if (kt < nk) kstep<false>(acc, R1, 0, kt);
    }
  }
};

#define CHAIN_MAX_HIDDEN 4
struct ChainHidden { const float *W, *bias, *gamma, *beta; float *z, *y, *stats; int K, ldw; };
struct ChainFwd {
  const float *A; int lda, M, nh;
  ChainHidden h[CHAIN_MAX_HIDDEN];
  const float *Wf, *bf; float *outf; int Nf, ldwf, ldof;
  float eps;
  const float *lat_eps; float *lat_out; const float *prop; int lat_Z, lat_ld, prop_w, prop_ld;
  unsigned long long *prof;
};
#define CHAIN_STAMP(i) do { if (P.prof && threadIdx.x == 0) P.prof[(size_t)blockIdx.x * 16 + (i)] = __builtin_amdgcn_s_memtime(); } while (0)

template <int MT>
__device__ __forceinline__ void chain_y_to_lds(float *yimg, const gf4 (&y)[MT][2], int li, int kq, int nw) {
#pragma unroll
  for (int a = 0; a < MT; a++)
#pragma unroll
    for (int b = 0; b < 2; b++) *reinterpret_cast<gf4 *>(yimg + (16 * a + li) * 256 + (((((nw + 16 * b) >> 2) + kq) ^ li) << 2)) = y[a][b];
}

template <int MT, int EPI, int FIN, bool LAT = false>
__global__ __launch_bounds__(CH_NT) void k_chain_fwd(const ChainFwd P) {
  using LD = ChainLds<MT>;
  constexpr int BM = LD::BM, NW = 8;
  extern __shared__ __attribute__((aligned(16))) float gemm_lds[];
  float *yimg = gemm_lds, *wst = gemm_lds + LD::YIMG, *red1 = wst + 2 * CH_WSTAGE, *red2 = red1 + BM * NW;
  const int t = threadIdx.x, lane = t & 63, wave = t >> 6, li = lane & 15, kq = lane >> 4, nw = wave * 32;
  const int m0 = blockIdx.x * BM, M = P.M;
  gf4 acc[MT][2];
  auto zero = [&]() {
#pragma unroll
    for (int a = 0; a < MT; a++)
#pragma unroll
      for (int b = 0; b < 2; b++) acc[a][b] = gf4{0.f, 0.f, 0.f, 0.f};
  };
  zero();
  int stamp = 0;
  CHAIN_STAMP(stamp++);
  {
    ChainGemm<MT, 2, true, false> G;
    G.init(P.A, P.lda, M, m0, P.h[0].W, P.h[0].ldw, 256, P.h[0].K, yimg, wst);
    G.early(); G.late(); G.loop(acc);
  }
  CHAIN_STAMP(stamp++);
  ChainGemm<MT, 2, true, true> G;
  ChainGemm<MT, 1, true, true> Gf;
  for (int l = 0;; l++) {
    const ChainHidden &H = P.h[l];
    const bool more = l + 1 < P.nh;
    if (more) { G.init(nullptr, 0, M, m0, P.h[l + 1].W, P.h[l + 1].ldw, 256, 256, yimg, wst, H.y); G.early(); }
    else if (FIN == 1) { Gf.init(nullptr, 0, M, m0, P.Wf, P.ldwf, P.Nf, 256, yimg, wst, H.y); Gf.early(); }
    gf4 bv[2], gv[2], bev[2];
#pragma unroll
    for (int b = 0; b < 2; b++) {
      const int col = nw + 16 * b + 4 * kq;
      bv[b] = *reinterpret_cast<const gf4 *>(H.bias + col);
      if (EPI == 1) { gv[b] = *reinterpret_cast<const gf4 *>(H.gamma + col); bev[b] = *reinterpret_cast<const gf4 *>(H.beta + col); }
    }
    float stat[MT];
#pragma unroll
    for (int a = 0; a < MT; a++) {
      const int row = m0 + 16 * a + li;
      float p = 0.f;
#pragma unroll
      for (int b = 0; b < 2; b++) {
        if (row < M) *reinterpret_cast<gf4 *>(H.z + (long long)row * 256 + nw + 16 * b + 4 * kq) = acc[a][b];
#pragma unroll
        for (int r = 0; r < 4; r++) { const float v = acc[a][b][r] + bv[b][r]; acc[a][b][r] = tm_silu(v); p += acc[a][b][r]; }
      }
      if (EPI == 1) { p += __shfl_xor(p, 16); stat[a] = p + __shfl_xor(p, 32); }
    }
    __syncthreads();
    if (EPI == 1) {
      auto exchange = [&](float *red) {
        if (kq == 0) {
#pragma unroll
          for (int a = 0; a < MT; a++) red[(16 * a + li) * NW + wave] = stat[a];
        }
        __syncthreads();
#pragma unroll
        for (int a = 0; a < MT; a++) {
          const gf4 *q = reinterpret_cast<const gf4 *>(red + (16 * a + li) * NW);
          float m = 0.f;
#pragma unroll
          for (int w4 = 0; w4 < NW / 4; w4++) { const gf4 v = q[w4]; m += (v.x + v.y) + (v.z + v.w); }
          stat[a] = m;
        }
      };
      exchange(red1);
      const float inv_n = 1.f / 256.f;
      float mean[MT];
#pragma unroll
      for (int a = 0; a < MT; a++) {
        mean[a] = stat[a] * inv_n;
        float q = 0.f;
#pragma unroll
        for (int b = 0; b < 2; b++)
#pragma unroll
          for (int r = 0; r < 4; r++) { acc[a][b][r] -= mean[a]; q += acc[a][b][r] * acc[a][b][r]; }
        q += __shfl_xor(q, 16);
        stat[a] = q + __shfl_xor(q, 32);
      }
      exchange(red2);
#pragma unroll
      for (int a = 0; a < MT; a++) {
        const int row = m0 + 16 * a + li;
        const float rstd = rsqrtf(stat[a] * inv_n + P.eps);
#pragma unroll
        for (int b = 0; b < 2; b++) acc[a][b] = acc[a][b] * rstd * gv[b] + bev[b];
        if (row < M && wave == 0 && kq == 0) { H.stats[2 * (long long)row] = mean[a]; H.stats[2 * (long long)row + 1] = rstd; }
      }
    }
    if (more || FIN == 1) chain_y_to_lds<MT>(yimg, acc, li, kq, nw);
    else {
#pragma unroll
      for (int a = 0; a < MT; a++) {
        const int row = m0 + 16 * a + li;
        if (row < M) {
#pragma unroll
          for (int b = 0; b < 2; b++) *reinterpret_cast<gf4 *>(H.y + (long long)row * 256 + nw + 16 * b + 4 * kq) = acc[a][b];
        }
      }
    }
    CHAIN_STAMP(stamp++);
    if (!more) break;
    zero();
    G.late(); G.loop(acc);
    CHAIN_STAMP(stamp++);
  }
  if (FIN == 1) {
    gf4 accf[MT][1];
#pragma unroll
    for (int a = 0; a < MT; a++) accf[a][0] = gf4{0.f, 0.f, 0.f, 0.f};
    Gf.late(); Gf.loop(accf);
    CHAIN_STAMP(stamp++);
    const int col = wave * 16 + 4 * kq;
    gf4 bvf = {0.f, 0.f, 0.f, 0.f};
    if (P.bf) {
#pragma unroll
      for (int r = 0; r < 4; r++) bvf[r] = col + r < P.Nf ? P.bf[col + r] : 0.f;
    }
    const bool vec = !(P.ldof & 3) && !((uintptr_t)P.outf & 15);
#pragma unroll
    for (int a = 0; a < MT; a++) {
      const int row = m0 + 16 * a + li;
      const gf4 v = accf[a][0] + bvf;
      if (row < M) {
        float *o = P.outf + (long long)row * P.ldof + col;
        if (vec && col + 3 < P.Nf) *reinterpret_cast<gf4 *>(o) = v;
        else {
#pragma unroll
          for (int r = 0; r < 4; r++) if (col + r < P.Nf) o[r] = v[r];
        }
      }
      if (LAT) accf[a][0] = v;
    }
    if (LAT) {
      float *ft = yimg;
      __syncthreads();
#pragma unroll
      for (int a = 0; a < MT; a++) *reinterpret_cast<gf4 *>(ft + (16 * a + li) * 128 + col) = accf[a][0];
      __syncthreads();
      const int Z = P.lat_Z, zq = Z >> 2;
      for (int it = t; it < BM * zq; it += CH_NT) {
        const int row = it / zq, q = it - row * zq;
        const long long gr = m0 + row;
        if (gr < M) {
          const gf4 mu = *reinterpret_cast<const gf4 *>(ft + row * 128 + 4 * q), lv = *reinterpret_cast<const gf4 *>(ft + row * 128 + Z + 4 * q);
          const gf4 ep = *reinterpret_cast<const gf4 *>(P.lat_eps + gr * Z + 4 * q);
          gf4 z;
#pragma unroll
          for (int r = 0; r < 4; r++) z[r] = fmaf(ep[r], expf(0.5f * lv[r]), mu[r]);
          *reinterpret_cast<gf4 *>(P.lat_out + gr * P.lat_ld + 4 * q) = z;
        }
      }
      const int ph = P.prop_w >> 1;
      for (int it = t; it < BM * ph; it += CH_NT) {
        const int row = it / ph, q = it - row * ph;
        const long long gr = m0 + row;
        if (gr < M) *reinterpret_cast<gf2 *>(P.lat_out + gr * P.lat_ld + Z + 2 * q) = *reinterpret_cast<const gf2 *>(P.prop + gr * P.prop_ld + 2 * q);
      }
    }
  }
  if (FIN == 2) {
    float *hs = wst;
    __syncthreads();
#pragma unroll
    for (int b = 0; b < 2; b++) {
      const gf4 wv = *reinterpret_cast<const gf4 *>(P.Wf + nw + 16 * b + 4 * kq);
#pragma unroll
      for (int a = 0; a < MT; a++) {
        float s = 0.f;
        s = fmaf(acc[a][b][0], wv[0], s); s = fmaf(acc[a][b][1], wv[1], s); s = fmaf(acc[a][b][2], wv[2], s); s = fmaf(acc[a][b][3], wv[3], s);
        hs[(16 * a + li) * 64 + 8 * wave + 4 * b + kq] = s;
      }
    }
    __syncthreads();
    if (t < BM && m0 + t < M) {
      float v[64];
#pragma unroll
      for (int g = 0; g < 64; g += 4) { const gf4 x = *reinterpret_cast<const gf4 *>(hs + t * 64 + g); v[g] = x.x; v[g + 1] = x.y; v[g + 2] = x.z; v[g + 3] = x.w; }
#pragma unroll
      for (int off = 32; off >= 1; off >>= 1)
#pragma unroll
        for (int g = 0; g < off; g++) v[g] = v[g] + v[g + off];
      P.outf[m0 + t] = v[0] + (P.bf ? P.bf[0] : 0.f);
    }
  }
  CHAIN_STAMP(stamp++);
}

struct ChainBwdStage {
  const float *W; int ldw;
  const float *z, *bias, *gamma, *stats;
  float *dz, *partial;
};
struct ChainBwd {
  const float *G; int ldg, Kg, M, ns;
  ChainBwdStage s[CHAIN_MAX_HIDDEN];
  const float *W0; int ldw0, dx_cols; float *dx; int lddx;
  unsigned long long *prof;
};

__device__ __forceinline__ void chain_o_to_lds(float *yimg, const float (&o)[8], int a, int li, int c0) {
  float *row = yimg + (16 * a + li) * 256;
  *reinterpret_cast<gf4 *>(row + ((((c0 >> 2)) ^ li) << 2)) = gf4{o[0], o[1], o[2], o[3]};
  *reinterpret_cast<gf4 *>(row + ((((c0 >> 2) + 1) ^ li) << 2)) = gf4{o[4], o[5], o[6], o[7]};
}

template <int MT, int EPI, bool HEAD, bool DX>
__global__ __launch_bounds__(CH_NT) void k_chain_bwd(const ChainBwd P) {
  using LD = ChainLds<MT>;
  constexpr int BM = LD::BM, NW = 8;
  extern __shared__ __attribute__((aligned(16))) float gemm_lds[];
  float *yimg = gemm_lds, *wst = gemm_lds + LD::YIMG, *red = wst + 2 * CH_WSTAGE;
  const int t = threadIdx.x, lane = t & 63, wave = t >> 6, li = lane & 15, kq = lane >> 4, nw = wave * 32;
  const int m0 = blockIdx.x * BM, M = P.M;
  const int c0 = nw + 8 * kq;
  gf4 acc[MT][2];
#define DY(a, j) acc[a][(j) & 1][(j) >> 1]
  auto zero = [&]() {
#pragma unroll
    for (int a = 0; a < MT; a++)
#pragma unroll
      for (int b = 0; b < 2; b++) acc[a][b] = gf4{0.f, 0.f, 0.f, 0.f};
  };
  int stamp = 0;
  CHAIN_STAMP(stamp++);
  if (HEAD) {
    float wv[8];
    { const gf4 w0 = *reinterpret_cast<const gf4 *>(P.s[0].W + c0), w1 = *reinterpret_cast<const gf4 *>(P.s[0].W + c0 + 4);
#pragma unroll
      for (int j = 0; j < 4; j++) { wv[j] = w0[j]; wv[4 + j] = w1[j]; } }
#pragma unroll
    for (int a = 0; a < MT; a++) {
      const int row = m0 + 16 * a + li;
      const float d = P.G[row < M ? row : M - 1];
#pragma unroll
      for (int j = 0; j < 8; j++) DY(a, j) = d * wv[j];
    }
  } else {
    zero();
    ChainGemm<MT, 2, false, false> G;
    G.init(P.G, P.ldg, M, m0, P.s[0].W, P.s[0].ldw, 256, P.Kg, yimg, wst);
    G.early(); G.late(); G.loop(acc);
  }
  CHAIN_STAMP(stamp++);
  ChainGemm<MT, 2, false, true> G;
  ChainGemm<MT, 1, false, true> Gx;
  for (int st = 0;; st++) {
    const ChainBwdStage &S = P.s[st];
    const bool more = st + 1 < P.ns;
    constexpr bool PRE = !(MT == 5 && (EPI == 2 || HEAD));
    if (more) { G.init(nullptr, 0, M, m0, P.s[st + 1].W, P.s[st + 1].ldw, 256, 256, yimg, wst, S.dz); if (PRE) G.early(); }
    else if (DX) { Gx.init(nullptr, 0, M, m0, P.W0, P.ldw0, P.dx_cols, 256, yimg, wst, S.dz); if (PRE) Gx.early(); }
    const bool keep = more || DX;
    float bv[8], gv[8];
    {
      const gf4 b0 = *reinterpret_cast<const gf4 *>(S.bias + c0), b1 = *reinterpret_cast<const gf4 *>(S.bias + c0 + 4);
#pragma unroll
      for (int j = 0; j < 4; j++) { bv[j] = b0[j]; bv[4 + j] = b1[j]; }
      if (EPI == 2) {
        const gf4 g0 = *reinterpret_cast<const gf4 *>(S.gamma + c0), g1 = *reinterpret_cast<const gf4 *>(S.gamma + c0 + 4);
#pragma unroll
        for (int j = 0; j < 4; j++) { gv[j] = g0[j]; gv[4 + j] = g1[j]; }
      }
    }
    if (EPI == 2) {
      float mean[MT], rstd[MT], m1[MT], m2[MT];
      const float inv_n = 1.f / 256.f;
#pragma unroll
      for (int a = 0; a < MT; a++) {
        const int row = m0 + 16 * a + li;
        const bool ok = row < M;
        const long long rr = ok ? row : M - 1;
        const gf4 z0 = *reinterpret_cast<const gf4 *>(S.z + rr * 256 + c0), z1 = *reinterpret_cast<const gf4 *>(S.z + rr * 256 + c0 + 4);
        mean[a] = S.stats[2 * rr]; rstd[a] = S.stats[2 * rr + 1];
        float s1 = 0.f, s2 = 0.f;
#pragma unroll
        for (int j = 0; j < 8; j++) {
          if (!ok) DY(a, j) = 0.f;
          const float v = (j < 4 ? z0[j] : z1[j - 4]) + bv[j];
          const float sig = tm_sigmoid(v), ah = (v * sig - mean[a]) * rstd[a], da = DY(a, j) * gv[j];
          s1 += da; s2 += da * ah;
        }
        s1 += __shfl_xor(s1, 16); s2 += __shfl_xor(s2, 16);
        m1[a] = s1 + __shfl_xor(s1, 32); m2[a] = s2 + __shfl_xor(s2, 32);
      }
      __syncthreads();
      if (kq == 0) {
#pragma unroll
        for (int a = 0; a < MT; a++) *reinterpret_cast<gf2 *>(red + ((16 * a + li) * NW + wave) * 2) = gf2{m1[a], m2[a]};
      }
      __syncthreads();
#pragma unroll
      for (int a = 0; a < MT; a++) {
        const gf4 *q = reinterpret_cast<const gf4 *>(red + (16 * a + li) * NW * 2);
        float t1 = 0.f, t2 = 0.f;
#pragma unroll
        for (int w4 = 0; w4 < NW / 2; w4++) { const gf4 x = q[w4]; t1 += x.x + x.z; t2 += x.y + x.w; }
        m1[a] = t1 * inv_n; m2[a] = t2 * inv_n;
      }
      float cg[8], cb[8], cz[8];
#pragma unroll
      for (int j = 0; j < 8; j++) { cg[j] = 0.f; cb[j] = 0.f; cz[j] = 0.f; }
#pragma unroll
      for (int a = 0; a < MT; a++) {
        const int row = m0 + 16 * a + li;
        const long long rr = row < M ? row : M - 1;
        const gf4 z0 = *reinterpret_cast<const gf4 *>(S.z + rr * 256 + c0), z1 = *reinterpret_cast<const gf4 *>(S.z + rr * 256 + c0 + 4);
        float o[8];
#pragma unroll
        for (int j = 0; j < 8; j++) {
          const float v = (j < 4 ? z0[j] : z1[j - 4]) + bv[j];
          const float sig = tm_sigmoid(v), ah = (v * sig - mean[a]) * rstd[a], da = DY(a, j) * gv[j];
          const float dact = rstd[a] * (da - m1[a] - ah * m2[a]);
          o[j] = dact * (sig * (1.f + v * (1.f - sig)));
          cg[j] += DY(a, j) * ah; cb[j] += DY(a, j); cz[j] += row < M ? o[j] : 0.f;
        }
        if (keep) chain_o_to_lds(yimg, o, a, li, c0);
        else if (row < M) {
          float *dst = S.dz + (long long)row * 256 + c0;
          *reinterpret_cast<gf4 *>(dst) = gf4{o[0], o[1], o[2], o[3]}; *reinterpret_cast<gf4 *>(dst + 4) = gf4{o[4], o[5], o[6], o[7]};
        }
      }
#pragma unroll
      for (int j = 0; j < 8; j++) { cg[j] = gemm_row16_sum(cg[j]); cb[j] = gemm_row16_sum(cb[j]); cz[j] = gemm_row16_sum(cz[j]); }
      if (li == 0) {
        float *pp = S.partial + (size_t)blockIdx.x * 3 * 256 + c0;
        *reinterpret_cast<gf4 *>(pp) = gf4{cg[0], cg[1], cg[2], cg[3]}; *reinterpret_cast<gf4 *>(pp + 4) = gf4{cg[4], cg[5], cg[6], cg[7]};
        *reinterpret_cast<gf4 *>(pp + 256) = gf4{cb[0], cb[1], cb[2], cb[3]}; *reinterpret_cast<gf4 *>(pp + 256 + 4) = gf4{cb[4], cb[5], cb[6], cb[7]};
        *reinterpret_cast<gf4 *>(pp + 512) = gf4{cz[0], cz[1], cz[2], cz[3]}; *reinterpret_cast<gf4 *>(pp + 512 + 4) = gf4{cz[4], cz[5], cz[6], cz[7]};
      }
    } else {
      if (keep) __syncthreads();
#pragma unroll
      for (int a = 0; a < MT; a++) {
        const int row = m0 + 16 * a + li;
        const long long rr = row < M ? row : M - 1;
        const gf4 z0 = *reinterpret_cast<const gf4 *>(S.z + rr * 256 + c0), z1 = *reinterpret_cast<const gf4 *>(S.z + rr * 256 + c0 + 4);
        float o[8];
#pragma unroll
        for (int j = 0; j < 8; j++) {
          const float x = (j < 4 ? z0[j] : z1[j - 4]) + bv[j], sig = tm_sigmoid(x);
          o[j] = DY(a, j) * (sig * (1.f + x * (1.f - sig)));
        }
        if (keep) chain_o_to_lds(yimg, o, a, li, c0);
        else if (row < M) {
          float *dst = S.dz + (long long)row * 256 + c0;
          *reinterpret_cast<gf4 *>(dst) = gf4{o[0], o[1], o[2], o[3]}; *reinterpret_cast<gf4 *>(dst + 4) = gf4{o[4], o[5], o[6], o[7]};
        }
      }
    }
    CHAIN_STAMP(stamp++);
    if (!more) break;
    zero();
    if (!PRE) G.early();
    G.late(); G.loop(acc);
    CHAIN_STAMP(stamp++);
  }
#undef DY
  if (DX) {
    gf4 accx[MT][1];
#pragma unroll
    for (int a = 0; a < MT; a++) accx[a][0] = gf4{0.f, 0.f, 0.f, 0.f};
    if (MT == 5 && EPI == 2) Gx.early();
    Gx.late(); Gx.loop(accx);
    CHAIN_STAMP(stamp++);
    const int col = wave * 16 + li;
#pragma unroll
    for (int a = 0; a < MT; a++)
#pragma unroll
      for (int r = 0; r < 4; r++) {
        const int row = m0 + 16 * a + 4 * kq + r;
        if (row < M && col < P.dx_cols) P.dx[(long long)row * P.lddx + col] = accx[a][0][r] + 0.f;
      }
  }
  CHAIN_STAMP(stamp++);
}
```

track_mjx_amd/csrc/tmjx_chain.hip:

```cpp
#include <hip/hip_runtime.h>

#include <stdlib.h>

#include <string>

#include "../../include/tmjx.h"
#include "mlp_chain.h"

extern "C" int tmjx_internal_fail(int code, const char *msg);
extern "C" int tmjx_internal_gemm_mt(int M, int col_tiles);
static int fail(int code, const std::string &msg) { return tmjx_internal_fail(code, msg.c_str()); }
static int check_launch(const char *what) {
  hipError_t e = hipGetLastError();
  if (e != hipSuccess) return fail(TMJX_EHIP, std::string(what) + ": " + hipGetErrorString(e));
  return TMJX_OK;
}
static bool al16(const void *p) { return !((uintptr_t)p & 15); }
static bool rows16(const void *p, long long ld) { return al16(p) && !(ld & 3); }

template <int MT, int EPI, int FIN, bool LAT = false>
static int launch_chain_fwd(const ChainFwd &P, hipStream_t s) {
  constexpr size_t lds = sizeof(float) * (size_t)ChainLds<MT>::TOTAL;
  static bool attr_set = false;
  if (!attr_set) {
    hipError_t e = hipFuncSetAttribute((const void *)k_chain_fwd<MT, EPI, FIN, LAT>, hipFuncAttributeMaxDynamicSharedMemorySize, (int)lds);
    if (e != hipSuccess) return fail(TMJX_EHIP, std::string("hipFuncSetAttribute(k_chain_fwd): ") + hipGetErrorString(e));
    attr_set = true;
  }
  hipLaunchKernelGGL((k_chain_fwd<MT, EPI, FIN, LAT>), dim3((P.M + 16 * MT - 1) / (16 * MT)), dim3(CH_NT), lds, s, P);
  return check_launch("k_chain_fwd");
}
template <int EPI, int FIN, bool LAT = false>
static int chain_fwd_mt(const ChainFwd &P, hipStream_t s) {
  if (tmjx_internal_gemm_mt(P.M, 1) == 2) return launch_chain_fwd<2, EPI, FIN, LAT>(P, s);
  return launch_chain_fwd<5, EPI, FIN, LAT>(P, s);
}

static int chain_rows(int M) { const int bm = 16 * tmjx_internal_gemm_mt(M, 1); return (M + bm - 1) / bm * bm; }
static const char *chain_fwd_why(const tmjx_chain_fwd_t *c) {
  if (!c || !c->A) return "null argument";
  if (c->M >= 1 && c->rows_alloc < chain_rows(c->M)) return "rows_alloc: the y buffers must hold tmjx_chain_rows(M) rows (whole row tiles are stored)";
  if (c->epi != 1 && c->epi != 3) return "epi must be 1 (Dense -> SiLU -> LayerNorm blocks) or 3 (Dense -> SiLU layers)";
  if (c->n_hidden < 1 || c->n_hidden > TMJX_CHAIN_MAX_HIDDEN) return "1 .. 4 hidden layers";
  if (c->M < 1 || !rows16(c->A, c->lda)) return "M >= 1 and 16-byte aligned input rows";
  for (int l = 0; l < c->n_hidden; l++) {
    const tmjx_chain_layer_t &h = c->hidden[l];
    if (!h.W || !h.bias || !h.z || !h.y || (c->epi == 1 && (!h.gamma || !h.beta || !h.stats))) return "null layer argument";
    if (h.K < 1 || h.ldw < h.K || !rows16(h.W, h.ldw) || !al16(h.bias) || !al16(h.z) || !al16(h.y)) return "layer operands must be 16-byte aligned with ldw >= K";
    if (c->epi == 1 && (!al16(h.gamma) || !al16(h.beta))) return "gamma / beta must be 16-byte aligned";
    if (l > 0 && h.K != 256) return "every hidden layer is 256 wide (layers behind the first have K = 256)";
    if (l == 0 && c->lda < h.K) return "lda < K of the first layer";
  }
  if (c->Wf) {
    if (!c->outf || c->Nf < 1 || c->Nf > 128) return "the last layer has 1 .. 128 columns";
    if (c->Nf == 1) { if (!al16(c->Wf)) return "the head's weight row must be 16-byte aligned"; }
    else if (c->ldwf < 256 || !rows16(c->Wf, c->ldwf) || c->ldof < c->Nf) return "the last layer's weight rows must be 16-byte aligned, ldwf >= 256, ldof >= Nf";
  }
  if (c->lat_out) {
    if (c->epi != 1 || !c->Wf || c->Nf != 2 * c->lat_Z || !c->lat_eps || !c->prop) return "the latent tail follows a LayerNorm-block chain whose last layer is [mean | logvar] (Nf = 2 lat_Z)";
    if (c->lat_Z < 4 || (c->lat_Z & 3) || c->prop_w < 0 || (c->prop_w & 1) || c->lat_ld < c->lat_Z + c->prop_w || (c->lat_ld & 3) || (c->prop_ld & 1) || c->prop_ld < c->prop_w)
      return "latent tail: lat_Z % 4 == 0, prop_w and prop_ld even, lat_ld % 4 == 0 and >= lat_Z + prop_w";
    if (!al16(c->lat_eps) || !al16(c->lat_out) || ((uintptr_t)c->prop & 7)) return "latent tail: lat_eps / lat_out 16-byte aligned, prop 8-byte aligned";
  }
  return nullptr;
}

template <int MT, int EPI, bool HEAD, bool DX>
static int launch_chain_bwd(const ChainBwd &P, hipStream_t s) {
  constexpr size_t lds = sizeof(float) * (size_t)ChainLds<MT>::TOTAL;
  static bool attr_set = false;
  if (!attr_set) {
    hipError_t e = hipFuncSetAttribute((const void *)k_chain_bwd<MT, EPI, HEAD, DX>, hipFuncAttributeMaxDynamicSharedMemorySize, (int)lds);
    if (e != hipSuccess) return fail(TMJX_EHIP, std::string("hipFuncSetAttribute(k_chain_bwd): ") + hipGetErrorString(e));
    attr_set = true;
  }
  hipLaunchKernelGGL((k_chain_bwd<MT, EPI, HEAD, DX>), dim3((P.M + 16 * MT - 1) / (16 * MT)), dim3(CH_NT), lds, s, P);
  return check_launch("k_chain_bwd");
}
template <int EPI, bool HEAD, bool DX>
static int chain_bwd_mt(const ChainBwd &P, hipStream_t s) {
  if (tmjx_internal_gemm_mt(P.M, 1) == 2) return launch_chain_bwd<2, EPI, HEAD, DX>(P, s);
  return launch_chain_bwd<5, EPI, HEAD, DX>(P, s);
}

static const char *chain_bwd_why(const tmjx_chain_bwd_t *c) {
  if (!c || !c->G) return "null argument";
  if (c->M >= 1 && c->rows_alloc < chain_rows(c->M)) return "rows_alloc: the dz buffers must hold tmjx_chain_rows(M) rows (whole row tiles are stored)";
  if (c->epi != 2 && c->epi != 4) return "epi must be 2 (Dense -> SiLU -> LayerNorm blocks) or 4 (Dense -> SiLU layers)";
  if (c->n_stages < 1 || c->n_stages > TMJX_CHAIN_MAX_HIDDEN) return "1 .. 4 stages (one per hidden layer)";
  if (c->M < 1 || c->Kg < 1 || c->Kg > 128) return "M >= 1 and a last layer of 1 .. 128 columns";
  const bool head = c->Kg == 1;
  if (head && c->epi != 4) return "a 1-wide last layer follows Dense -> SiLU layers (epi 4) only";
  if (!head && (c->ldg < c->Kg || (c->Kg & 3) || !rows16(c->G, c->ldg))) return "the output gradient's rows must be 16-byte aligned with Kg % 4 == 0";
  for (int l = 0; l < c->n_stages; l++) {
    const tmjx_chain_bwd_stage_t &s = c->stage[l];
    if (!s.W || !s.z || !s.bias || !s.dz || (c->epi == 2 && (!s.gamma || !s.stats || !s.partial))) return "null stage argument";
    if (!al16(s.W) || !al16(s.z) || !al16(s.bias) || !al16(s.dz) || (c->epi == 2 && (!al16(s.gamma) || !al16(s.partial)))) return "stage operands must be 16-byte aligned";
    if (!(head && l == 0) && (s.ldw < 256 || (s.ldw & 3))) return "weight rows must be 16-byte aligned with ldw >= 256";
  }
  if (c->W0) {
    if (head) return "no trailing input gradient behind a 1-wide head's chain";
    if (!c->dx || c->dx_cols < 1 || c->dx_cols > 128 || c->lddx < c->dx_cols || !rows16(c->W0, c->ldw0) || c->ldw0 < ((c->dx_cols + 3) & ~3)) return "the trailing input gradient has 1 .. 128 columns, W0 rows 16-byte aligned";
  }
  return nullptr;
}

extern "C" {
int tmjx_chain_rows(int M) { return M < 1 ? 0 : chain_rows(M); }
int tmjx_chain_bwd_ok(const tmjx_chain_bwd_t *c) { return chain_bwd_why(c) == nullptr; }
int tmjx_chain_bwd(const tmjx_chain_bwd_t *c, void *stream) {
  if (const char *why = chain_bwd_why(c)) return fail(TMJX_EINVAL, std::string("tmjx_chain_bwd: ") + why);
  ChainBwd P{};
  P.G = c->G; P.ldg = c->ldg; P.Kg = c->Kg; P.M = c->M; P.ns = c->n_stages;
  for (int l = 0; l < c->n_stages; l++) {
    const tmjx_chain_bwd_stage_t &s = c->stage[l];
    P.s[l] = ChainBwdStage{s.W, s.ldw, s.z, s.bias, s.gamma, s.stats, s.dz, s.partial};
  }
  P.W0 = c->W0; P.ldw0 = c->ldw0; P.dx_cols = c->dx_cols; P.dx = c->dx; P.lddx = c->lddx;
  P.prof = (unsigned long long *)c->prof;
  hipStream_t s = (hipStream_t)stream;
  if (c->epi == 2) return c->W0 ? chain_bwd_mt<2, false, true>(P, s) : chain_bwd_mt<2, false, false>(P, s);
  if (c->Kg == 1) return chain_bwd_mt<4, true, false>(P, s);
  return c->W0 ? chain_bwd_mt<4, false, true>(P, s) : chain_bwd_mt<4, false, false>(P, s);
}
int tmjx_chain_fwd_ok(const tmjx_chain_fwd_t *c) { return chain_fwd_why(c) == nullptr; }
int tmjx_chain_fwd(const tmjx_chain_fwd_t *c, void *stream) {
  if (const char *why = chain_fwd_why(c)) return fail(TMJX_EINVAL, std::string("tmjx_chain_fwd: ") + why);
  ChainFwd P{};
  P.A = c->A; P.lda = c->lda; P.M = c->M; P.nh = c->n_hidden; P.eps = c->eps;
  for (int l = 0; l < c->n_hidden; l++) {
    const tmjx_chain_layer_t &h = c->hidden[l];
    P.h[l] = ChainHidden{h.W, h.bias, h.gamma, h.beta, h.z, h.y, h.stats, h.K, h.ldw};
  }
  P.Wf = c->Wf; P.bf = c->bf; P.outf = c->outf; P.Nf = c->Nf; P.ldwf = c->ldwf; P.ldof = c->ldof;
  P.prof = (unsigned long long *)c->prof;
  P.lat_eps = c->lat_eps; P.lat_out = c->lat_out; P.prop = c->prop; P.lat_Z = c->lat_Z; P.lat_ld = c->lat_ld; P.prop_w = c->prop_w; P.prop_ld = c->prop_ld;
  hipStream_t s = (hipStream_t)stream;
  const int fin = !c->Wf ? 0 : (c->Nf == 1 ? 2 : 1);
  if (c->epi == 1) {
    if (fin == 0) return chain_fwd_mt<1, 0>(P, s);
    if (fin == 1 && c->lat_out) return chain_fwd_mt<1, 1, true>(P, s);
    if (fin == 1) return chain_fwd_mt<1, 1>(P, s);
    return fail(TMJX_EINVAL, "tmjx_chain_fwd: a 1-wide last layer follows Dense -> SiLU layers (epi 3) only");
  }
  if (fin == 0) return chain_fwd_mt<3, 0>(P, s);
  if (fin == 2) return chain_fwd_mt<3, 2>(P, s);
  return chain_fwd_mt<3, 1>(P, s);
}
}
```

track_mjx_amd/hip.py:

```python
from __future__ import annotations

import ctypes as C
import os
import subprocess
from pathlib import Path

_PKG = Path(__file__).resolve().parent
SO_PATH = Path(os.environ.get("TMJX_SO", str(_PKG / "libtmjx_hip.so")))
CSRC = _PKG / "csrc"
SOURCES = (CSRC / "tmjx_hip.hip", CSRC / "tmjx_bf16.hip", CSRC / "tmjx_wave.hip", CSRC / "tmjx_chain.hip")
SOURCE_FLAGS = {"tmjx_wave.hip": ("-mllvm", "-disable-machine-licm")}


class TmjxError(RuntimeError):
    pass


class Layout(C.Structure):
    _fields_ = [(n, C.c_int32) for n in (
        "nq", "nv", "nu", "nbody", "ncon", "nefc", "obs_size", "ref_obs_size", "n_metrics", "window",
        "qpos", "qvel", "act", "qacc_warmstart", "time", "xpos", "xmat_torso", "qfrc_actuator",
        "prev_ctrl", "action_buffer", "done", "steps_f", "first_phys", "first_obs", "first_prev_ctrl", "state_rows",
        "i_clip_idx", "i_start_frame", "i_buffer_index", "i_nan_count", "istate_rows", "ws_rows")]


EXPORTS = ("tmjx_model_create", "tmjx_model_destroy", "tmjx_layout", "tmjx_clips_upload", "tmjx_reset", "tmjx_step",
           "tmjx_physics", "tmjx_physics_step", "tmjx_forward", "tmjx_reward_obs", "tmjx_reward_frame", "tmjx_gae", "tmjx_ppo_scratch_floats", "tmjx_ppo_loss", "tmjx_ppo_loss_phases",
           "tmjx_silu_ln_partial_floats", "tmjx_silu_ln_fwd", "tmjx_silu_ln_bwd", "tmjx_silu_ln_fwd_bf16", "tmjx_silu_ln_bwd_bf16", "tmjx_minibatch_begin_bf16", "tmjx_gather_normalize", "tmjx_latent_concat", "tmjx_latent_concat_bwd", "tmjx_latent_concat_bwd_add", "tmjx_sample_action", "tmjx_linear_nolds", "tmjx_linear_act", "tmjx_linear_act_ok", "tmjx_linear_nolds_norm", "tmjx_linear_nolds_bf16", "tmjx_adam_clip", "tmjx_adam_clip_norm", "tmjx_adam_norm_floats", "tmjx_colsum_scratch_floats", "tmjx_colsum",
           "tmjx_gather_minibatch", "tmjx_minibatch_begin", "tmjx_philox4x32_10", "tmjx_gemm_nt", "tmjx_gemm_nt_silu_ln", "tmjx_gemm_nt_silu_ln_ok", "tmjx_gemm_nn", "tmjx_colsum_grouped", "tmjx_gemm_nn_ln_bwd", "tmjx_gemm_nn_ln_bwd_ok", "tmjx_gemm_nn_ln_bwd_partial_floats", "tmjx_gemm_dw", "tmjx_gemm_dw_grouped", "tmjx_gemm_dw_grouped_wgs", "tmjx_gemm_dw_scratch_floats", "tmjx_set_wrappers", "tmjx_set_action_repeat", "tmjx_stats_scratch_floats", "tmjx_stats_sums", "tmjx_stats_apply",
           "tmjx_rollout_store", "tmjx_clips_share", "tmjx_gemm_nt_silu", "tmjx_gemm_nt_silu_ok", "tmjx_silu_fwd", "tmjx_silu_bwd", "tmjx_gemm_nn_silu_bwd_ok", "tmjx_gemm_nn_silu_bwd", "tmjx_silu_bwd_rank1", "tmjx_head_dw_scratch_floats", "tmjx_head_dw", "tmjx_head_fwd_ok", "tmjx_head_fwd", "tmjx_bf16_shadow", "tmjx_bgemm_nt", "tmjx_bgemm_dw", "tmjx_bgemm_dw_grouped", "tmjx_bgemm_dw_scratch_floats", "tmjx_bgemm_row_tile_ok", "tmjx_bf16_z_bytes", "tmjx_bgemm_partial_floats",
           "tmjx_bgemm_ln_fwd", "tmjx_bgemm_ln_bwd", "tmjx_bgemm_silu_fwd", "tmjx_bgemm_silu_bwd", "tmjx_bf_silu_bwd", "tmjx_bf_silu_bwd_rank1",
           "tmjx_chain_rows", "tmjx_chain_fwd_ok", "tmjx_chain_fwd", "tmjx_chain_bwd_ok", "tmjx_chain_bwd",
           "tmjx_debug_rows", "tmjx_last_error", "tmjx_version")


class Minibatch(C.Structure):
    _fields_ = ([(k, C.c_void_p) for k in ("obs", "next_last", "raw_action", "log_prob", "reward", "discount", "truncation", "perm", "mean", "std", "obs_n", "next_n",
                                           "raw_action_g", "scalars_g", "eps", "noise", "state")] + [("seed", C.c_uint64)] +
                [(k, C.c_int32) for k in ("T", "R", "B", "W", "A", "Z", "advance")])


class ColsumProblem(C.Structure):
    _fields_ = [("partial", C.c_void_p), ("out", C.c_void_p), ("rows", C.c_int32), ("width", C.c_int32)]


class DwProblem(C.Structure):
    _fields_ = [("dY", C.c_void_p), ("X", C.c_void_p), ("dW", C.c_void_p), ("db", C.c_void_p), ("scratch", C.c_void_p),
                ("ldy", C.c_int32), ("ldx", C.c_int32), ("lddw", C.c_int32), ("M", C.c_int32), ("N", C.c_int32), ("K", C.c_int32)]


class BdwProblem(C.Structure):
    _fields_ = [("dY", C.c_void_p), ("X", C.c_void_p), ("dW", C.c_void_p), ("db", C.c_void_p), ("scratch", C.c_void_p),
                ("y_is_f32", C.c_int32), ("x_is_f32", C.c_int32), ("ldy", C.c_int32), ("ldx", C.c_int32), ("lddw", C.c_int32), ("M", C.c_int32), ("N", C.c_int32), ("K", C.c_int32)]


class RolloutStore(C.Structure):
    _fields_ = [(k, C.c_void_p) for k in ("obs", "obs_dst0", "obs_dst1", "raw", "raw_dst", "logp", "logp_dst", "reward", "reward_dst", "done", "discount_dst",
                                          "trunc", "trunc_dst")] + [(k, C.c_int32) for k in ("n", "W", "A")] + [("obs_dst2", C.c_void_p)]


class Bf16Shadow(C.Structure):
    _fields_ = [("src", C.c_void_p), ("dst", C.c_void_p), ("dst_t", C.c_void_p), ("N", C.c_int32), ("K", C.c_int32), ("ld_src", C.c_int32),
                ("ld_dst", C.c_int32), ("ld_dst_t", C.c_int32)]


class ChainLayer(C.Structure):
    _fields_ = [(k, C.c_void_p) for k in ("W", "bias", "gamma", "beta", "z", "y", "stats")] + [("K", C.c_int32), ("ldw", C.c_int32)]


class ChainFwd(C.Structure):
    _fields_ = [("A", C.c_void_p), ("lda", C.c_int32), ("M", C.c_int32), ("n_hidden", C.c_int32), ("epi", C.c_int32), ("hidden", ChainLayer * 4),
                ("Wf", C.c_void_p), ("bf", C.c_void_p), ("outf", C.c_void_p), ("Nf", C.c_int32), ("ldwf", C.c_int32), ("ldof", C.c_int32), ("eps", C.c_float), ("rows_alloc", C.c_int32),
                ("lat_eps", C.c_void_p), ("lat_out", C.c_void_p), ("prop", C.c_void_p), ("lat_Z", C.c_int32), ("lat_ld", C.c_int32), ("prop_w", C.c_int32), ("prop_ld", C.c_int32),
                ("prof", C.c_void_p)]


class ChainBwdStage(C.Structure):
    _fields_ = [("W", C.c_void_p), ("ldw", C.c_int32)] + [(k, C.c_void_p) for k in ("z", "bias", "gamma", "stats", "dz", "partial")]


class ChainBwd(C.Structure):
    _fields_ = [("G", C.c_void_p), ("ldg", C.c_int32), ("Kg", C.c_int32), ("M", C.c_int32), ("n_stages", C.c_int32), ("epi", C.c_int32), ("stage", ChainBwdStage * 4),
                ("W0", C.c_void_p), ("ldw0", C.c_int32), ("dx_cols", C.c_int32), ("dx", C.c_void_p), ("lddx", C.c_int32), ("rows_alloc", C.c_int32), ("prof", C.c_void_p)]


class PpoCfg(C.Structure):
    _fields_ = [("T", C.c_int32), ("B", C.c_int32), ("A", C.c_int32), ("Z", C.c_int32), ("reward_scaling", C.c_float),
                ("discounting", C.c_float), ("gae_lambda", C.c_float), ("clip_eps", C.c_float), ("entropy_cost", C.c_float),
                ("kl_weight", C.c_float), ("normalize_advantage", C.c_int32), ("accumulate", C.c_int32)]

_lib = None


def build(verbose: bool = False, out: Path | None = None, defines: tuple = ()) -> Path:
    out = SO_PATH if out is None else Path(out)
    import hashlib
    import re
    from concurrent.futures import ThreadPoolExecutor
    flags = ["--offload-arch=gfx950", "-O3", "-std=c++17", "-fno-slp-vectorize", "-fPIC", "-Wno-unused-value", *[f"-D{d}" for d in defines],
             *os.environ.get("TMJX_EXTRA_HIPCC_FLAGS", "").split()]

    def closure(path: Path, seen: dict) -> dict:
        if path in seen or not path.exists():
            return seen
        text = path.read_text()
        seen[path] = text
        for inc in re.findall(r'^\s*#\s*include\s+"([^"]+)"', text, re.M):
            closure((path.parent / inc).resolve(), seen)
        return seen

    cache = out.parent / ".build"
    cache.mkdir(exist_ok=True)
    objs = []
    def flags_of(src):
        return [*flags, *SOURCE_FLAGS.get(src.name, ())]

    for src in SOURCES:
        h = hashlib.sha256(" ".join(flags_of(src)).encode())
        for pth, text in sorted(closure(src.resolve(), {}).items()):
            h.update(str(pth.name).encode()); h.update(text.encode())
        objs.append(cache / f"{src.stem}.{h.hexdigest()[:16]}.o")

    def compile_one(src, obj):
        if obj.exists():
            return
        for stale in cache.glob(f"{src.stem}.*.o"):
            if len(list(cache.glob(f"{src.stem}.*.o"))) > 6:
                stale.unlink(missing_ok=True)
        tmp = obj.with_suffix(f".tmp{os.getpid()}.o")
        cmd = ["hipcc", *flags_of(src), "-c", "-o", str(tmp), str(src)]
        res = subprocess.run(cmd, capture_output=True, text=True)
        if res.returncode != 0:
            raise TmjxError(f"hipcc failed on {src.name}:\n" + res.stderr[-4000:])
        tmp.replace(obj)
        if verbose:
            print(" ".join(cmd))
    with ThreadPoolExecutor(len(SOURCES)) as ex:
        for f in [ex.submit(compile_one, s, o) for s, o in zip(SOURCES, objs)]:
            f.result()
    cmd = ["hipcc", "--offload-arch=gfx950", "-shared", "-fPIC", "-o", str(out), *[str(o) for o in objs]]
    res = subprocess.run(cmd, capture_output=True, text=True)
    if res.returncode != 0:
        raise TmjxError("hipcc link failed:\n" + res.stderr[-4000:])
    Path(str(out) + ".id").write_text(hashlib.sha256(" ".join(o.name for o in objs).encode()).hexdigest()[:16] + "\n")
    return out


def build_id(path: Path | None = None) -> str:
    import hashlib
    path = Path(SO_PATH if path is None else path)
    side = Path(str(path) + ".id")
    try:
        if side.exists() and side.stat().st_mtime >= path.stat().st_mtime - 1:
            return side.read_text().strip()
        return hashlib.sha256(path.read_bytes()).hexdigest()[:16]
    except OSError:
        return "missing"


def lib():
    global _lib
    if _lib is not None:
        return _lib
    _lib = load(SO_PATH)
    return _lib


def load(path: Path):
    path = Path(path)
    if not path.exists():
        raise TmjxError(f"{path} is missing: build it with `python -c 'import __graft_entry__ as g; g.build()'` "
                        "(hipcc --offload-arch=gfx950). There is no CPU fallback for the hot path.")
    try:
        L = C.CDLL(str(path))
    except OSError as e:
        raise TmjxError(f"cannot load {path}: {e}") from e
    vp, ip, fp = C.c_void_p, C.POINTER(C.c_int32), C.c_void_p
    sig: dict = {}
    sig.setdefault("tmjx_model_create", [None, None])[0] = [C.c_char_p, C.c_size_t, C.POINTER(vp)]
    sig.setdefault("tmjx_model_destroy", [None, None])[0] = [vp]
    sig.setdefault("tmjx_model_destroy", [None, None])[1] = None
    sig.setdefault("tmjx_layout", [None, None])[0] = [vp, C.POINTER(Layout)]
    sig.setdefault("tmjx_clips_upload", [None, None])[0] = [vp, vp, vp, vp, vp, vp, C.c_int, C.c_int]
    sig.setdefault("tmjx_reset", [None, None])[0] = [vp, fp, vp, vp, vp, fp, fp, fp, fp, C.c_int, vp]
    sig.setdefault("tmjx_step", [None, None])[0] = [vp, fp, vp, fp, fp, fp, fp, fp, fp, fp, C.c_int, vp]
    sig.setdefault("tmjx_physics", [None, None])[0] = [vp, fp, fp, C.c_int, fp, C.c_int, vp]
    sig.setdefault("tmjx_physics_step", [None, None])[0] = [vp, fp, fp, fp, C.c_int, vp]
    sig.setdefault("tmjx_forward", [None, None])[0] = [vp, fp, fp, C.c_int, vp]
    sig.setdefault("tmjx_reward_obs", [None, None])[0] = [vp, fp, vp, fp, fp, fp, fp, fp, fp, fp, C.c_int, vp]
    sig.setdefault("tmjx_reward_frame", [None, None])[0] = [vp, fp, vp, fp] + [fp] * 5 + [fp] * 5 + [C.c_int, vp]
    sig.setdefault("tmjx_gae", [None, None])[0] = [fp, fp, fp, fp, fp, C.c_float, C.c_float, fp, fp, C.c_int, C.c_int, vp]
    sig.setdefault("tmjx_ppo_scratch_floats", [None, None])[0] = [C.c_int, C.c_int]
    sig.setdefault("tmjx_ppo_loss", [None, None])[0] = [C.POINTER(PpoCfg)] + [fp] * 15 + [vp]
    sig.setdefault("tmjx_ppo_loss_phases", [None, None])[0] = [C.POINTER(PpoCfg)] + [fp] * 15 + [C.c_int, vp]
    sig.setdefault("tmjx_silu_ln_partial_floats", [None, None])[0] = [C.c_int, C.c_int]
    sig.setdefault("tmjx_silu_ln_fwd", [None, None])[0] = [fp] * 6 + [C.c_int, C.c_int, C.c_float, vp]
    sig.setdefault("tmjx_silu_ln_bwd", [None, None])[0] = [fp] * 8 + [C.c_int, C.c_int, vp]
    sig.setdefault("tmjx_silu_ln_fwd_bf16", [None, None])[0] = [fp] * 5 + [C.c_int, fp, C.c_int, C.c_int, C.c_float, vp]
    sig.setdefault("tmjx_silu_ln_bwd_bf16", [None, None])[0] = [fp] * 6 + [C.c_int, fp, fp, C.c_int, C.c_int, vp]
    sig.setdefault("tmjx_gather_normalize", [None, None])[0] = [fp] * 5 + [C.c_int] * 4 + [vp]
    sig.setdefault("tmjx_gather_minibatch", [None, None])[0] = [fp] * 14 + [C.c_int] * 5 + [vp]
    sig.setdefault("tmjx_minibatch_begin", [None, None])[0] = [C.POINTER(Minibatch), vp]
    sig.setdefault("tmjx_minibatch_begin_bf16", [None, None])[0] = [C.POINTER(Minibatch), fp, C.c_int, vp]
    sig.setdefault("tmjx_philox4x32_10", [None, None])[0] = [fp, fp, vp]
    sig.setdefault("tmjx_latent_concat", [None, None])[0] = [fp] * 4 + [C.c_int] * 4 + [C.c_int64, C.c_int64, fp, fp, C.c_int, C.c_uint64, fp, vp]
    sig.setdefault("tmjx_latent_concat_bwd", [None, None])[0] = [fp] * 4 + [C.c_int] * 3 + [vp]
    sig.setdefault("tmjx_latent_concat_bwd_add", [None, None])[0] = [fp] * 5 + [C.c_int] * 3 + [vp]
    sig.setdefault("tmjx_sample_action", [None, None])[0] = [fp] * 5 + [C.c_int, C.c_int, C.c_uint64, fp, vp]
    sig.setdefault("tmjx_linear_nolds", [None, None])[0] = [fp, C.c_int64, C.c_int64, fp, fp, fp, C.c_int, C.c_int, C.c_int, vp]
    sig.setdefault("tmjx_linear_act", [None, None])[0] = [fp, C.c_int64, fp, C.c_int, fp, fp, C.c_int, C.c_int, C.c_int, fp, fp, vp]
    sig.setdefault("tmjx_linear_act_ok", [None, None])[0] = [fp, C.c_int64, fp, C.c_int, C.c_int]
    sig.setdefault("tmjx_linear_nolds_norm", [None, None])[0] = [fp, C.c_int64, C.c_int64, fp, fp, fp, C.c_int, C.c_int, C.c_int, fp, fp, vp]
    sig.setdefault("tmjx_linear_nolds_bf16", [None, None])[0] = [fp, C.c_int64, C.c_int64, fp, C.c_int, fp, fp, C.c_int, C.c_int, C.c_int, fp, fp, vp]
    sig.setdefault("tmjx_colsum_scratch_floats", [None, None])[0] = [C.c_int]
    sig.setdefault("tmjx_colsum", [None, None])[0] = [fp, fp, fp, C.c_int, C.c_int, vp]
    sig.setdefault("tmjx_adam_clip", [None, None])[0] = [fp] * 5 + [C.c_longlong] + [C.c_float] * 7 + [vp]
    sig.setdefault("tmjx_adam_clip_norm", [None, None])[0] = [fp] * 6 + [C.c_longlong] + [C.c_float] * 7 + [vp]
    sig.setdefault("tmjx_gemm_nt", [None, None])[0] = [fp, C.c_int, fp, C.c_int, fp, fp, C.c_int, C.c_int, C.c_int, C.c_int, vp]
    sig.setdefault("tmjx_gemm_nt_silu_ln_ok", [None, None])[0] = [fp, C.c_int, fp, C.c_int, C.c_int]
    sig.setdefault("tmjx_gemm_nt_silu_ln", [None, None])[0] = [fp, C.c_int, fp, C.c_int, fp, fp, fp, fp, fp, C.c_int, fp, C.c_int, C.c_int, C.c_int, C.c_float, vp]
    sig.setdefault("tmjx_colsum_grouped", [None, None])[0] = [C.POINTER(ColsumProblem), C.c_int, vp]
    sig.setdefault("tmjx_gemm_nn_ln_bwd_ok", [None, None])[0] = [fp, C.c_int, fp, C.c_int, C.c_int]
    sig.setdefault("tmjx_gemm_nn_ln_bwd_partial_floats", [None, None])[0] = [C.c_int, C.c_int]
    sig.setdefault("tmjx_gemm_nn_ln_bwd_partial_floats", [None, None])[1] = C.c_longlong
    sig.setdefault("tmjx_gemm_nn_ln_bwd", [None, None])[0] = [fp, C.c_int, fp, C.c_int, fp, fp, fp, fp, fp, fp, C.c_int, C.c_int, C.c_int, vp]
    sig.setdefault("tmjx_gemm_nn", [None, None])[0] = [fp, C.c_int, fp, C.c_int, fp, C.c_int, C.c_int, C.c_int, C.c_int, vp]
    sig.setdefault("tmjx_gemm_dw_scratch_floats", [None, None])[0] = [C.c_int, C.c_int, C.c_int]
    sig.setdefault("tmjx_gemm_dw_scratch_floats", [None, None])[1] = C.c_longlong
    sig.setdefault("tmjx_gemm_dw", [None, None])[0] = [fp, C.c_int, fp, C.c_int, fp, fp, fp, C.c_int, C.c_int, C.c_int, vp]
    sig.setdefault("tmjx_gemm_dw_grouped", [None, None])[0] = [C.POINTER(DwProblem), C.c_int, vp]
    sig.setdefault("tmjx_gemm_dw_grouped_wgs", [None, None])[0] = [C.POINTER(DwProblem), C.c_int, C.c_int, vp]
    sig.setdefault("tmjx_gemm_nt_silu_ok", [None, None])[0] = [fp, C.c_int, fp, C.c_int]
    sig.setdefault("tmjx_gemm_nt_silu", [None, None])[0] = [fp, C.c_int, fp, C.c_int, fp, fp, fp, C.c_int, C.c_int, C.c_int, C.c_int, vp]
    sig.setdefault("tmjx_silu_fwd", [None, None])[0] = [fp, fp, fp, C.c_longlong, C.c_int, vp]
    sig.setdefault("tmjx_silu_bwd", [None, None])[0] = [fp, fp, fp, fp, C.c_longlong, C.c_int, vp]
    sig.setdefault("tmjx_gemm_nn_silu_bwd_ok", [None, None])[0] = [fp, C.c_int, fp, C.c_int]
    sig.setdefault("tmjx_gemm_nn_silu_bwd", [None, None])[0] = [fp, C.c_int, fp, C.c_int, fp, fp, fp, C.c_int, C.c_int, C.c_int, vp]
    sig.setdefault("tmjx_silu_bwd_rank1", [None, None])[0] = [fp, fp, fp, fp, fp, C.c_longlong, C.c_int, vp]
    sig.setdefault("tmjx_head_dw_scratch_floats", [None, None])[0] = [C.c_int, C.c_int]
    sig.setdefault("tmjx_head_dw_scratch_floats", [None, None])[1] = C.c_longlong
    sig.setdefault("tmjx_head_dw", [None, None])[0] = [fp, fp, C.c_int, fp, fp, fp, C.c_int, C.c_int, vp]
    sig.setdefault("tmjx_head_fwd_ok", [None, None])[0] = [fp, C.c_int, fp, C.c_int]
    sig.setdefault("tmjx_head_fwd", [None, None])[0] = [fp, C.c_int, fp, fp, fp, C.c_int, C.c_int, vp]
    sig.setdefault("tmjx_rollout_store", [None, None])[0] = [C.POINTER(RolloutStore), vp]
    sig.setdefault("tmjx_clips_share", [None, None])[0] = [vp, vp]
    sig.setdefault("tmjx_bf16_shadow", [None, None])[0] = [C.POINTER(Bf16Shadow), C.c_int, vp]
    sig.setdefault("tmjx_bgemm_nt", [None, None])[0] = [fp, C.c_int, C.c_int, fp, C.c_int, fp, fp, C.c_int, C.c_int, C.c_int, C.c_int, vp]
    sig.setdefault("tmjx_bgemm_row_tile_ok", [None, None])[0] = [C.c_int]
    sig.setdefault("tmjx_bgemm_partial_floats", [None, None])[0] = [C.c_int, C.c_int, C.c_int]
    sig.setdefault("tmjx_bgemm_partial_floats", [None, None])[1] = C.c_longlong
    sig.setdefault("tmjx_bgemm_ln_fwd", [None, None])[0] = [fp, C.c_int, C.c_int, fp, C.c_int, fp, fp, fp, fp, C.c_int, fp, C.c_int, fp, C.c_int, C.c_int, C.c_int, C.c_float, vp]
    sig.setdefault("tmjx_bgemm_ln_bwd", [None, None])[0] = [fp, C.c_int, C.c_int, fp, C.c_int, fp, C.c_int, fp, fp, fp, fp, C.c_int, fp, C.c_int, C.c_int, C.c_int, vp]
    sig.setdefault("tmjx_bgemm_silu_fwd", [None, None])[0] = [fp, C.c_int, C.c_int, fp, C.c_int, fp, fp, C.c_int, fp, C.c_int, fp, C.c_int, C.c_int, C.c_int, C.c_int, vp]
    sig.setdefault("tmjx_bgemm_silu_bwd", [None, None])[0] = [fp, C.c_int, C.c_int, fp, C.c_int, fp, C.c_int, fp, fp, C.c_int, fp, C.c_int, C.c_int, C.c_int, vp]
    sig.setdefault("tmjx_bf_silu_bwd", [None, None])[0] = [fp, C.c_int, fp, C.c_int, fp, fp, C.c_int, fp, C.c_int, C.c_int, vp]
    sig.setdefault("tmjx_bf_silu_bwd_rank1", [None, None])[0] = [fp, fp, fp, C.c_int, fp, fp, C.c_int, fp, C.c_int, C.c_int, vp]
    sig.setdefault("tmjx_bgemm_dw_scratch_floats", [None, None])[0] = [C.c_int, C.c_int, C.c_int]
    sig.setdefault("tmjx_bgemm_dw_scratch_floats", [None, None])[1] = C.c_longlong
    sig.setdefault("tmjx_bgemm_dw", [None, None])[0] = [fp, C.c_int, C.c_int, fp, C.c_int, C.c_int, fp, C.c_int, fp, fp, C.c_int, C.c_int, C.c_int, vp]
    sig.setdefault("tmjx_bgemm_dw_grouped", [None, None])[0] = [C.POINTER(BdwProblem), C.c_int, C.c_int, vp]
    sig.setdefault("tmjx_set_wrappers", [None, None])[0] = [vp, C.c_int, C.c_int]
    sig.setdefault("tmjx_set_action_repeat", [None, None])[0] = [vp, C.c_int]
    sig.setdefault("tmjx_stats_scratch_floats", [None, None])[0] = [C.c_int]
    sig.setdefault("tmjx_stats_sums", [None, None])[0] = [fp, fp, fp, fp, C.c_longlong, C.c_int, vp]
    sig.setdefault("tmjx_stats_apply", [None, None])[0] = [fp, C.c_float, fp, fp, fp, fp, C.c_int, C.c_float, C.c_float, vp]
    sig.setdefault("tmjx_chain_rows", [None, None])[0] = [C.c_int]
    sig.setdefault("tmjx_chain_fwd_ok", [None, None])[0] = [C.POINTER(ChainFwd)]
    sig.setdefault("tmjx_chain_fwd", [None, None])[0] = [C.POINTER(ChainFwd), vp]
    sig.setdefault("tmjx_chain_bwd_ok", [None, None])[0] = [C.POINTER(ChainBwd)]
    sig.setdefault("tmjx_chain_bwd", [None, None])[0] = [C.POINTER(ChainBwd), vp]
    sig.setdefault("tmjx_debug_rows", [None, None])[0] = [vp, C.c_char_p, ip, ip]
    sig.setdefault("tmjx_last_error", [None, None])[1] = C.c_char_p
    sig.setdefault("tmjx_version", [None, None])[1] = C.c_char_p
    restype_set = {"tmjx_model_destroy"}
    for name, (argtypes, restype) in sig.items():
        fn = getattr(L, name, None)
        if fn is None:
            continue
        if argtypes is not None:
            fn.argtypes = argtypes
        if restype is not None or name in restype_set:
            fn.restype = restype
    return L


def check(rc: int, what: str) -> None:
    if rc != 0:
        raise TmjxError(f"{what} failed ({rc}): {lib().tmjx_last_error().decode()}")


def block_override() -> str | None:
    return os.environ.get("TMJX_BLOCK")
```

Measured before the change: 1.694 million.

## Fold latent reparameterization backward into encoder chain backward GEMM A-load

The latent concat backward no longer launches its own kernel when a fold object is present. It parks its arguments, and the encoder's chain backward kernel computes the fc2 gradient (mean part plus eps*0.5*exp(0.5*logvar) part plus the pending add) while loading A tiles, writing dfc2 out as it goes. This removes a separate kernel launch and a round trip of the fc2 gradient through memory. The fused path only applies for small-M tile configs and otherwise falls back to the old separate kernel. It also adds a backward-compatibility check in _f32_chain_ok, per-device LDS attribute caching, and disables the fast k-loop path for the latent variant.

```diff
diff --git a/include/tmjx.h b/include/tmjx.h
--- a/include/tmjx.h
+++ b/include/tmjx.h
@@ -181,6 +181,7 @@
   const float *W0; int32_t ldw0, dx_cols; float *dx; int32_t lddx;
   int32_t rows_alloc;
   void *prof;
+  const float *lat_dx, *lat_eps, *lat_fc2, *lat_add; int32_t lat_Z, lat_ldx;
 } tmjx_chain_bwd_t;
 int tmjx_chain_bwd_ok(const tmjx_chain_bwd_t *chain);
 int tmjx_chain_bwd(const tmjx_chain_bwd_t *chain, void *stream);
diff --git a/track_mjx_amd/agent/networks.py b/track_mjx_amd/agent/networks.py
--- a/track_mjx_amd/agent/networks.py
+++ b/track_mjx_amd/agent/networks.py
@@ -395,7 +395,7 @@
     return bool(_hip.lib().tmjx_chain_fwd_ok(C.byref(chain_fwd_desc(x2[:1], hidden, final, kind)[0])))
 
 
-def chain_bwd(g, final_w, blocks, kind="ln", w0=None, dx_cols=None, prof=None, dx_ld=None):
+def chain_bwd(g, final_w, blocks, kind="ln", w0=None, dx_cols=None, prof=None, dx_ld=None, lat=None):
     import ctypes as C
     from .. import hip as _hip
     L = _hip.lib()
@@ -424,6 +424,11 @@
         d.W0, d.ldw0, d.dx_cols, d.dx, d.lddx = w0.data_ptr(), w0.stride(0), cols, dx.data_ptr(), dx.stride(0)
     if prof is not None:
         d.prof = prof.data_ptr()
+    if lat is not None:
+        ldx, leps, lfc2, ladd = lat
+        d.lat_dx, d.lat_ldx, d.lat_eps, d.lat_fc2, d.lat_Z = ldx.data_ptr(), ldx.stride(0), leps.data_ptr(), lfc2.data_ptr(), leps.shape[1]
+        if ladd is not None:
+            d.lat_add = ladd.data_ptr()
     _launch("tmjx_chain_bwd", dev, C.byref(d))
     return dzs, (partials if kind == "ln" else None), dx
 
@@ -603,7 +608,7 @@
 class _F32ChainFn(torch.autograd.Function):
 
     @staticmethod
-    def forward(ctx, x, layers, dx_cols, latent, *params):
+    def forward(ctx, x, layers, dx_cols, latent, fold, *params):
         x2 = _rows2d(x)
         hid, last = layers[:-1], layers[-1]
         kind = hid[0].kind
@@ -618,7 +623,7 @@
         saved, out = chain_fwd(x2, hidden, (last.lin.weight, last.lin.bias), kind, eps, latent=latent)
         flat = [t for z, y, st in saved for t in ((z, y, st) if kind == "ln" else (z, y))]
         ctx.save_for_backward(x2, *flat, *params)
-        ctx.layers, ctx.dx_cols, ctx.x_shape, ctx.kind, ctx.nflat = layers, dx_cols, x.shape, kind, len(flat)
+        ctx.layers, ctx.dx_cols, ctx.x_shape, ctx.kind, ctx.nflat, ctx.fold = layers, dx_cols, x.shape, kind, len(flat), fold
         res = out.view(*x.shape[:-1], last.lin.out_features) if last.kind == "dense" else out.view(*x.shape[:-1], 1)
         if dec_in is None:
             return res
@@ -644,6 +649,7 @@
         grads: dict = {}
         wf, bf = P[-1][0], P[-1][1]
         y_last = saved[-1][1]
+        lat = ctx.fold.take(dout) if ctx.fold is not None else None
         if last.kind == "head":
             g = dout.reshape(-1)
             g = g if g.is_contiguous() else g.contiguous()
@@ -658,15 +664,21 @@
             if g.data_ptr() % 16 or g.stride(0) % 4:
                 g = g.contiguous()
             got = d.try_add(g, y_last, last.lin.weight, last.lin.bias) if d is not None else None
-            dw, db = got if got is not None else gemm_dw(g, y_last, True)
-            grads[(len(layers) - 1, 0)], grads[(len(layers) - 1, 1)] = dw, db
+            if got is not None or lat is None:
+                dw, db = got if got is not None else gemm_dw(g, y_last, True)
+                grads[(len(layers) - 1, 0)], grads[(len(layers) - 1, 1)] = dw, db
         if kind == "ln":
             blocks = [(P[l][0], saved[l][0], P[l][1], P[l][2], saved[l][2]) for l in range(len(hid) - 1, -1, -1)]
         else:
             blocks = [(P[l][0], saved[l][0], P[l][1]) for l in range(len(hid) - 1, -1, -1)]
         want_dx = ctx.needs_input_grad[0]
         cols = (x2.shape[1] if ctx.dx_cols is None else int(ctx.dx_cols)) if want_dx else None
-        dzs, partials, dx = chain_bwd(g, wf, blocks, kind, P[0][0] if want_dx else None, cols, dx_ld=x2.shape[1] if want_dx else None)
+        if lat is not None:
+            dzs, partials, dx = chain_bwd(g, wf, blocks, kind, P[0][0] if want_dx else None, cols, dx_ld=x2.shape[1] if want_dx else None, lat=lat)
+            if (len(layers) - 1, 0) not in grads:
+                grads[(len(layers) - 1, 0)], grads[(len(layers) - 1, 1)] = gemm_dw(g, y_last, True)
+        else:
+            dzs, partials, dx = chain_bwd(g, wf, blocks, kind, P[0][0] if want_dx else None, cols, dx_ld=x2.shape[1] if want_dx else None)
         for i, dz in enumerate(dzs):
             l = len(hid) - 1 - i
             L = hid[l]
@@ -686,12 +698,55 @@
                 got = d.try_add(dz, xin, L.lin.weight, L.lin.bias) if d is not None else None
                 grads[(l, 0)], grads[(l, 1)] = got if got is not None else gemm_dw(dz, xin, True)
         out = [grads.get((l, j)) for l, L in enumerate(layers) for j in range(len(L.params()))]
-        return (dx.view(ctx.x_shape) if dx is not None else None, None, None, None, *out)
-
-
-def f32_chain(x, layers, dx_cols=None, latent=None):
+        return (dx.view(ctx.x_shape) if dx is not None else None, None, None, None, None, *out)
+
+
+def f32_chain(x, layers, dx_cols=None, latent=None, fold=None):
     params = [p for L in layers for p in L.params()]
-    return _F32ChainFn.apply(x, layers, dx_cols, latent, *params)
+    return _F32ChainFn.apply(x, layers, dx_cols, latent, fold, *params)
+
+
+class _LatentFold:
+    __slots__ = ("buf", "args")
+
+    def __init__(self):
+        self.buf, self.args = None, None
+
+    def park(self, dfc2, dx, eps, fc2, add):
+        self.buf, self.args = dfc2, (dx, eps, fc2, add)
+
+    def take(self, dout):
+        buf, args = self.buf, self.args
+        self.buf, self.args = None, None
+        if buf is None:
+            return None
+        if dout is None or dout.data_ptr() != buf.data_ptr() or dout.numel() != buf.numel():
+            raise RuntimeError("_LatentFold: fc2 received a gradient besides the latent sample's and the KL term's (the folded backward cannot add it)")
+        return args
+
+
+def _chain_bwd_ok(layers, kind, dx_cols) -> bool:
+    import ctypes as C
+    from .. import hip as _hip
+    hid, last = layers[:-1], layers[-1]
+    stand = hid[0].lin.weight.data_ptr() // 16 * 16 or 16
+    d = _hip.ChainBwd()
+    head = last.kind == "head"
+    Kg = 1 if head else last.lin.out_features
+    d.G, d.ldg, d.Kg, d.M, d.n_stages, d.epi = stand, (1 if head else (Kg + 3) // 4 * 4), Kg, 1, len(hid), 2 if kind == "ln" else 4
+    d.rows_alloc = int(_hip.lib().tmjx_chain_rows(1))
+    for i in range(len(hid)):
+        w = last.lin.weight if i == 0 else hid[len(hid) - i].lin.weight
+        L = hid[len(hid) - 1 - i]
+        S = d.stage[i]
+        S.W, S.ldw = w.data_ptr(), (w.stride(0) if w.dim() == 2 and w.shape[0] > 1 else 256)
+        S.z, S.bias, S.dz = stand, L.lin.bias.data_ptr(), stand
+        if kind == "ln":
+            S.gamma, S.stats, S.partial = L.norm.weight.data_ptr(), stand, stand
+    if dx_cols is not None:
+        w0 = hid[0].lin.weight
+        d.W0, d.ldw0, d.dx_cols, d.dx, d.lddx = w0.data_ptr(), w0.stride(0), int(dx_cols), stand, (int(dx_cols) + 3) // 4 * 4
+    return bool(_hip.lib().tmjx_chain_bwd_ok(C.byref(d)))
 
 
 def _f32_chain_ok(x, layers, dx_cols=None) -> bool:
@@ -704,7 +759,12 @@
         return False
     kind = hid[0].kind
     hidden = [(L.lin.weight, L.lin.bias, L.norm.weight, L.norm.bias) if kind == "ln" else (L.lin.weight, L.lin.bias) for L in hid]
-    return chain_fwd_ok(_rows2d(x), hidden, (last.lin.weight, last.lin.bias), kind)
+    if not chain_fwd_ok(_rows2d(x), hidden, (last.lin.weight, last.lin.bias), kind):
+        return False
+    if torch.is_grad_enabled() and (x.requires_grad or any(p.requires_grad for L in layers for p in L.params())):
+        want_dx = x.requires_grad
+        return _chain_bwd_ok(layers, kind, (x.shape[-1] if dx_cols is None else int(dx_cols)) if want_dx else None)
+    return True
 
 
 class _BlockLink:
@@ -1103,10 +1163,10 @@
 class _LatentConcatFn(torch.autograd.Function):
 
     @staticmethod
-    def forward(ctx, fc2, eps, obs, ref, handle=None):
+    def forward(ctx, fc2, eps, obs, ref, handle=None, fold=None):
         import ctypes as C
         from .. import hip as _hip
-        ctx.handle = handle
+        ctx.handle, ctx.fold = handle, fold
         n, Z = eps.shape
         W = obs.shape[1]
         fc2, eps, obs = fc2.contiguous(), eps.contiguous(), obs.contiguous()
@@ -1131,26 +1191,30 @@
         add = ctx.handle.take() if ctx.handle is not None else None
         if add is not None and (add.shape != fc2.shape or not add.is_contiguous()):
             raise RuntimeError("_LatentConcatFn: the pending fc2 gradient does not fit this forward pass")
+        fold = getattr(ctx, "fold", None)
+        if fold is not None and add is not None and dx.stride(0) % 2 == 0 and dx.data_ptr() % 8 == 0 and add.data_ptr() % 16 == 0:
+            fold.park(dfc2, dx, eps, fc2, add)
+            return dfc2, None, None, None, None, None
         with torch.cuda.device(fc2.device):
             stream = C.c_void_p(torch.cuda.current_stream(fc2.device).cuda_stream)
             if add is None:
                 _hip.check(_hip.lib().tmjx_latent_concat_bwd(p(dx), p(eps), p(fc2), p(dfc2), n, Z, dx.shape[1], stream), "tmjx_latent_concat_bwd")
             else:
                 _hip.check(_hip.lib().tmjx_latent_concat_bwd_add(p(dx), p(eps), p(fc2), p(add), p(dfc2), n, Z, dx.shape[1], stream), "tmjx_latent_concat_bwd_add")
-        return dfc2, None, None, None, None
+        return dfc2, None, None, None, None, None
 
 
 class _LatentViewFn(torch.autograd.Function):
 
     @staticmethod
-    def forward(ctx, fc2, eps, x, handle=None):
-        ctx.handle = handle
+    def forward(ctx, fc2, eps, x, handle=None, fold=None):
+        ctx.handle, ctx.fold = handle, fold
         ctx.save_for_backward(fc2.contiguous(), eps.contiguous())
         return x.view_as(x)
 
     @staticmethod
     def backward(ctx, dx):
-        return (_LatentConcatFn.backward(ctx, dx)[0], None, None, None)
+        return (_LatentConcatFn.backward(ctx, dx)[0], None, None, None, None)
 
 
 class LatentGradHandle:
@@ -1200,6 +1264,7 @@
             raise RuntimeError("IntentionPolicy: the fc2 gradient parked on the previous forward pass (LatentGradHandle.add) was never consumed by a "
                                "backward pass through that forward — it would have been dropped")
         chains = _bf16_chain_ok(obs) and all(m.out_features % 4 == 0 for m in (self.fc2, self.head))
+        fold = None
         if chains:
             if getattr(self, "_enc_chain", None) is None:
                 self._enc_chain = [_Layer("ln", b.dense, b.norm) for b in self.encoder] + [_Layer("dense", self.fc2)]
@@ -1211,6 +1276,7 @@
                 self._dec_f32 = [_Layer("ln", b.dense, b.norm) for b in self.decoder] + [_Layer("dense", self.head)]
             xlat = None
             if obs.is_cuda and _f32_chain_ok(traj, self._enc_f32):
+                fold = _LatentFold()
                 obs2 = obs.reshape(-1, obs.shape[-1])
                 if (not deterministic and obs.dtype == torch.float32 and obs2.shape[0] * 2 * self.latents >= 2 * self.latents * 1024 and self.latents % 4 == 0
                         and (obs.shape[-1] - self.reference_obs_size) % 2 == 0 and obs2.stride(1) == 1 and obs2.stride(0) % 2 == 0 and self.reference_obs_size % 2 == 0
@@ -1218,9 +1284,9 @@
                     if eps is None:
                         eps = torch.randn(obs.shape[:-1] + (self.latents,), dtype=torch.float32, device=obs.device)
                     eps2 = eps.reshape(-1, self.latents).contiguous()
-                    fc2, xlat = f32_chain(traj, self._enc_f32, latent=(eps2, obs2[:, self.reference_obs_size:]))
+                    fc2, xlat = f32_chain(traj, self._enc_f32, latent=(eps2, obs2[:, self.reference_obs_size:]), fold=fold)
                 else:
-                    fc2 = f32_chain(traj, self._enc_f32)
+                    fc2 = f32_chain(traj, self._enc_f32, fold=fold)
             else:
                 with ln_bwd_links():
                     h = self.encoder(traj)
@@ -1233,9 +1299,10 @@
                 eps = torch.randn_like(mean)
             handle = LatentGradHandle(fc2.reshape(-1, fc2.shape[-1])) if (fc2.requires_grad and fc2.is_contiguous()) else None
             if not chains and xlat is not None:
-                x = _LatentViewFn.apply(fc2.reshape(-1, fc2.shape[-1]), eps.reshape(-1, self.latents), xlat, handle)
+                x = _LatentViewFn.apply(fc2.reshape(-1, fc2.shape[-1]), eps.reshape(-1, self.latents), xlat, handle, fold)
             else:
-                x = _LatentConcatFn.apply(fc2.reshape(-1, fc2.shape[-1]), eps.reshape(-1, self.latents), obs.reshape(-1, obs.shape[-1]), self.reference_obs_size, handle)
+                x = _LatentConcatFn.apply(fc2.reshape(-1, fc2.shape[-1]), eps.reshape(-1, self.latents), obs.reshape(-1, obs.shape[-1]), self.reference_obs_size, handle,
+                                          fold)
             self.latent_grad_handle = handle
             x = x.view(*lead, x.shape[-1])
             if chains:
diff --git a/track_mjx_amd/csrc/mlp_chain.h b/track_mjx_amd/csrc/mlp_chain.h
--- a/track_mjx_amd/csrc/mlp_chain.h
+++ b/track_mjx_amd/csrc/mlp_chain.h
@@ -9,20 +9,23 @@
   static_assert(2 * (BM + 8) * GEMM_LDA <= YIMG, "the first layer's A stages live in the Y image region");
 };
 
-template <int MT, int NI, bool BT, bool A_LDS>
+template <int MT, int NI, bool BT, bool A_LDS, bool LATG = false>
 struct ChainGemm {
   static constexpr int BM = 16 * MT, BN = 128 * NI, A_ROWS = BM + 8;
   static constexpr int A_PASS = A_LDS ? 0 : (BM * 8 + CH_NT - 1) / CH_NT, B_PASS = BN / 64, NPASS = A_PASS + B_PASS;
   static constexpr int LDB_N = BN + 4, A_STAGE = A_ROWS * GEMM_LDA;
   static constexpr int NMFMA = 4 * MT * NI, NFR = MT + (BT ? NI : 4 * NI);
   static constexpr int SPREAD = (NMFMA - NFR) / (NPASS + 1) > 0 ? (NMFMA - NFR) / (NPASS + 1) : 1;
-  struct Stage { gf4 v[NPASS]; int m[NPASS]; };
+  struct LatNone {};
+  struct LatRegs { gf4 e[A_PASS > 0 ? A_PASS : 1], l[A_PASS > 0 ? A_PASS : 1], d[A_PASS > 0 ? A_PASS : 1]; int k0; };
+  struct Stage { gf4 v[NPASS]; int m[NPASS]; std::conditional_t<LATG, LatRegs, LatNone> x; };
   struct Frag { gf4 a[MT], b[NI]; };
   static constexpr int T4 = A_LDS ? BM / 8 : 0, TRK = MT >= 4 ? 2 : 1;
   const float *A, *W;
   float *ast, *yimg, *wst, *tr_dst;
   int lda, ldw, M, N, K, m0, t, li, kq, nw;
   const float *pa[A_PASS > 0 ? A_PASS : 1], *pb[B_PASS];
+  const float *ldx, *leps, *lfc2, *ladd; float *ldst; int lZ, lldx;
   Stage R0, R1;
   Frag F0, F1;
 
@@ -42,7 +45,27 @@
       else { const int r = f / (BN / 4), c4 = f % (BN / 4); pb[p] = W + (long long)r * ldw + min(4 * c4, ((N + 3) & ~3) - 4); }
     }
   }
+  __device__ __forceinline__ void lat(const float *dx_, int ldx_, const float *eps_, const float *fc2_, const float *add_, float *dfc2_, int Z_) {
+    ldx = dx_; lldx = ldx_; leps = eps_; lfc2 = fc2_; ladd = add_; ldst = dfc2_; lZ = Z_;
+  }
   __device__ __forceinline__ void gload(Stage &R, int k0) {
+    if constexpr (LATG) {
+      R.x.k0 = k0;
+#pragma unroll
+      for (int p = 0; p < A_PASS; p++) {
+        const int f = t + CH_NT * p, r = f >> 3, c = k0 + 4 * (f & 7);
+        const bool in = f < BM * 8 && m0 + r < M && c < K, lv = in && c >= lZ;
+        const long long row = m0 + (in ? r : 0);
+        const int cz = lv ? c - lZ : (in ? c : 0);
+        R.m[p] = in ? (lv ? 2 : 1) : 0;
+        const float *q = ldx + row * lldx + cz;
+        const gf2 a = *reinterpret_cast<const gf2 *>(q), b = *reinterpret_cast<const gf2 *>(q + 2);
+        R.v[p] = gf4{a.x, a.y, b.x, b.y};
+        R.x.e[p] = *reinterpret_cast<const gf4 *>(leps + row * lZ + (lv ? cz : 0));
+        R.x.l[p] = *reinterpret_cast<const gf4 *>(lfc2 + row * K + (lv ? c : 0));
+        R.x.d[p] = ladd ? *reinterpret_cast<const gf4 *>(ladd + row * K + (in ? c : 0)) : gf4{0.f, 0.f, 0.f, 0.f};
+      }
+    } else
 #pragma unroll
     for (int p = 0; p < A_PASS; p++) {
       const int f = t + CH_NT * p, r = f >> 3, c4 = f & 7;
@@ -74,6 +97,21 @@
 #pragma unroll
     for (int p = 0; p < A_PASS; p++) {
       const int f = t + CH_NT * p, r = f < BM * 8 ? f >> 3 : BM + ((f >> 3) & 7), c4 = f & 7;
+      if constexpr (LATG) {
+        gf4 o = {0.f, 0.f, 0.f, 0.f};
+        if (R.m[p]) {
+#pragma unroll
+          for (int j = 0; j < 4; j++) {
+#pragma clang fp contract(off)
+            const float g = R.v[p][j];
+            float gm = g, gv = g * R.x.e[p][j] * (0.5f * expf(0.5f * R.x.l[p][j]));
+            if (ladd) { gm = R.x.d[p][j] + gm; gv = R.x.d[p][j] + gv; }
+            o[j] = R.m[p] == 1 ? gm : gv;
+          }
+          *reinterpret_cast<gf4 *>(ldst + (long long)(m0 + r) * K + R.x.k0 + 4 * c4) = o;
+        }
+        *reinterpret_cast<gf4 *>(sa + r * GEMM_LDA + 4 * c4) = o;
+      } else
       *reinterpret_cast<gf4 *>(sa + r * GEMM_LDA + 4 * c4) = MASKED ? gemm_mask4(R.v[p], R.m[p]) : R.v[p];
     }
 #pragma unroll
@@ -175,7 +213,7 @@
     }
     const int nk = (K + GEMM_BK - 1) / GEMM_BK;
     int kt = 0;
-    const int nfast = (A_LDS || (K % GEMM_BK) == 0) ? nk : max(0, (nk - 4) & ~1);
+    const int nfast = LATG ? 0 : (A_LDS || (K % GEMM_BK) == 0) ? nk : max(0, (nk - 4) & ~1);
     for (; kt + 1 < nfast; kt += 2) { kstep<true>(acc, R1, 0, kt); kstep<true>(acc, R0, 1, kt + 1); }
     if (kt < nfast) { kstep<true>(acc, R1, 0, kt); kt = nk; }
     if constexpr (!A_LDS) {
@@ -406,6 +444,7 @@
   ChainBwdStage s[CHAIN_MAX_HIDDEN];
   const float *W0; int ldw0, dx_cols; float *dx; int lddx;
   unsigned long long *prof;
+  const float *lat_dx, *lat_eps, *lat_fc2, *lat_add; int lat_Z, lat_ldx;
 };
 
 __device__ __forceinline__ void chain_o_to_lds(float *yimg, const float (&o)[8], int a, int li, int c0) {
@@ -414,7 +453,7 @@
   *reinterpret_cast<gf4 *>(row + ((((c0 >> 2) + 1) ^ li) << 2)) = gf4{o[4], o[5], o[6], o[7]};
 }
 
-template <int MT, int EPI, bool HEAD, bool DX>
+template <int MT, int EPI, bool HEAD, bool DX, bool LAT = false>
 __global__ __launch_bounds__(CH_NT) void k_chain_bwd(const ChainBwd P) {
   using LD = ChainLds<MT>;
   constexpr int BM = LD::BM, NW = 8;
@@ -447,8 +486,9 @@
     }
   } else {
     zero();
-    ChainGemm<MT, 2, false, false> G;
+    ChainGemm<MT, 2, false, false, LAT> G;
     G.init(P.G, P.ldg, M, m0, P.s[0].W, P.s[0].ldw, 256, P.Kg, yimg, wst);
+    if constexpr (LAT) G.lat(P.lat_dx, P.lat_ldx, P.lat_eps, P.lat_fc2, P.lat_add, const_cast<float *>(P.G), P.lat_Z);
     G.early(); G.late(); G.loop(acc);
   }
   CHAIN_STAMP(stamp++);
diff --git a/track_mjx_amd/csrc/tmjx_chain.hip b/track_mjx_amd/csrc/tmjx_chain.hip
--- a/track_mjx_amd/csrc/tmjx_chain.hip
+++ b/track_mjx_amd/csrc/tmjx_chain.hip
@@ -18,15 +18,23 @@
 static bool al16(const void *p) { return !((uintptr_t)p & 15); }
 static bool rows16(const void *p, long long ld) { return al16(p) && !(ld & 3); }
 
+#define CH_MAX_DEVICES 64
+static int lds_attr(bool (&set)[CH_MAX_DEVICES], const void *kern, size_t lds, const char *what) {
+  int dev = 0;
+  hipError_t e = hipGetDevice(&dev);
+  if (e != hipSuccess) return fail(TMJX_EHIP, std::string("hipGetDevice: ") + hipGetErrorString(e));
+  if (dev >= 0 && dev < CH_MAX_DEVICES && set[dev]) return TMJX_OK;
+  e = hipFuncSetAttribute(kern, hipFuncAttributeMaxDynamicSharedMemorySize, (int)lds);
+  if (e != hipSuccess) return fail(TMJX_EHIP, std::string("hipFuncSetAttribute(") + what + "): " + hipGetErrorString(e));
+  if (dev >= 0 && dev < CH_MAX_DEVICES) set[dev] = true;
+  return TMJX_OK;
+}
+
 template <int MT, int EPI, int FIN, bool LAT = false>
 static int launch_chain_fwd(const ChainFwd &P, hipStream_t s) {
   constexpr size_t lds = sizeof(float) * (size_t)ChainLds<MT>::TOTAL;
-  static bool attr_set = false;
-  if (!attr_set) {
-    hipError_t e = hipFuncSetAttribute((const void *)k_chain_fwd<MT, EPI, FIN, LAT>, hipFuncAttributeMaxDynamicSharedMemorySize, (int)lds);
-    if (e != hipSuccess) return fail(TMJX_EHIP, std::string("hipFuncSetAttribute(k_chain_fwd): ") + hipGetErrorString(e));
-    attr_set = true;
-  }
+  static bool attr_set[CH_MAX_DEVICES] = {};
+  if (int rc = lds_attr(attr_set, (const void *)k_chain_fwd<MT, EPI, FIN, LAT>, lds, "k_chain_fwd")) return rc;
   hipLaunchKernelGGL((k_chain_fwd<MT, EPI, FIN, LAT>), dim3((P.M + 16 * MT - 1) / (16 * MT)), dim3(CH_NT), lds, s, P);
   return check_launch("k_chain_fwd");
 }
@@ -65,22 +73,18 @@
   return nullptr;
 }
 
-template <int MT, int EPI, bool HEAD, bool DX>
+template <int MT, int EPI, bool HEAD, bool DX, bool LAT>
 static int launch_chain_bwd(const ChainBwd &P, hipStream_t s) {
   constexpr size_t lds = sizeof(float) * (size_t)ChainLds<MT>::TOTAL;
-  static bool attr_set = false;
-  if (!attr_set) {
-    hipError_t e = hipFuncSetAttribute((const void *)k_chain_bwd<MT, EPI, HEAD, DX>, hipFuncAttributeMaxDynamicSharedMemorySize, (int)lds);
-    if (e != hipSuccess) return fail(TMJX_EHIP, std::string("hipFuncSetAttribute(k_chain_bwd): ") + hipGetErrorString(e));
-    attr_set = true;
-  }
-  hipLaunchKernelGGL((k_chain_bwd<MT, EPI, HEAD, DX>), dim3((P.M + 16 * MT - 1) / (16 * MT)), dim3(CH_NT), lds, s, P);
+  static bool attr_set[CH_MAX_DEVICES] = {};
+  if (int rc = lds_attr(attr_set, (const void *)k_chain_bwd<MT, EPI, HEAD, DX, LAT>, lds, "k_chain_bwd")) return rc;
+  hipLaunchKernelGGL((k_chain_bwd<MT, EPI, HEAD, DX, LAT>), dim3((P.M + 16 * MT - 1) / (16 * MT)), dim3(CH_NT), lds, s, P);
   return check_launch("k_chain_bwd");
 }
 template <int EPI, bool HEAD, bool DX>
 static int chain_bwd_mt(const ChainBwd &P, hipStream_t s) {
-  if (tmjx_internal_gemm_mt(P.M, 1) == 2) return launch_chain_bwd<2, EPI, HEAD, DX>(P, s);
-  return launch_chain_bwd<5, EPI, HEAD, DX>(P, s);
+  if (tmjx_internal_gemm_mt(P.M, 1) == 2) return launch_chain_bwd<2, EPI, HEAD, DX, false>(P, s);
+  return launch_chain_bwd<5, EPI, HEAD, DX, false>(P, s);
 }
 
 static const char *chain_bwd_why(const tmjx_chain_bwd_t *c) {
@@ -92,6 +96,13 @@
   const bool head = c->Kg == 1;
   if (head && c->epi != 4) return "a 1-wide last layer follows Dense -> SiLU layers (epi 4) only";
   if (!head && (c->ldg < c->Kg || (c->Kg & 3) || !rows16(c->G, c->ldg))) return "the output gradient's rows must be 16-byte aligned with Kg % 4 == 0";
+  if (c->lat_dx) {
+    if (c->epi != 2 || head || c->W0 || c->Kg != 2 * c->lat_Z || c->ldg != c->Kg || !c->lat_eps || !c->lat_fc2)
+      return "the folded latent gradient: a LayerNorm-block chain (epi 2) without W0 behind fc2 = [mean | logvar] (Kg = 2 lat_Z, ldg = Kg)";
+    if (c->lat_Z < 4 || (c->lat_Z & 3) || c->lat_ldx < c->lat_Z || (c->lat_ldx & 1) || ((uintptr_t)c->lat_dx & 7) || !al16(c->lat_eps) || !al16(c->lat_fc2) ||
+        (c->lat_add && !al16(c->lat_add)))
+      return "the folded latent gradient: lat_Z % 4 == 0, lat_dx 8-byte aligned with an even lat_ldx >= lat_Z, lat_eps / lat_fc2 / lat_add 16-byte aligned";
+  }
   for (int l = 0; l < c->n_stages; l++) {
     const tmjx_chain_bwd_stage_t &s = c->stage[l];
     if (!s.W || !s.z || !s.bias || !s.dz || (c->epi == 2 && (!s.gamma || !s.stats || !s.partial))) return "null stage argument";
@@ -118,7 +129,16 @@
   }
   P.W0 = c->W0; P.ldw0 = c->ldw0; P.dx_cols = c->dx_cols; P.dx = c->dx; P.lddx = c->lddx;
   P.prof = (unsigned long long *)c->prof;
+  P.lat_dx = c->lat_dx; P.lat_eps = c->lat_eps; P.lat_fc2 = c->lat_fc2; P.lat_add = c->lat_add; P.lat_Z = c->lat_Z; P.lat_ldx = c->lat_ldx;
   hipStream_t s = (hipStream_t)stream;
+  if (c->epi == 2 && c->lat_dx) {
+    if (tmjx_internal_gemm_mt(P.M, 1) == 2) return launch_chain_bwd<2, 2, false, false, true>(P, s);
+    const int rc = c->lat_add ? tmjx_latent_concat_bwd_add(c->lat_dx, c->lat_eps, c->lat_fc2, c->lat_add, const_cast<float *>(c->G), c->M, c->lat_Z, c->lat_ldx, stream)
+                              : tmjx_latent_concat_bwd(c->lat_dx, c->lat_eps, c->lat_fc2, const_cast<float *>(c->G), c->M, c->lat_Z, c->lat_ldx, stream);
+    if (rc != TMJX_OK) return rc;
+    P.lat_dx = nullptr;
+    return chain_bwd_mt<2, false, false>(P, s);
+  }
   if (c->epi == 2) return c->W0 ? chain_bwd_mt<2, false, true>(P, s) : chain_bwd_mt<2, false, false>(P, s);
   if (c->Kg == 1) return chain_bwd_mt<4, true, false>(P, s);
   return c->W0 ? chain_bwd_mt<4, false, true>(P, s) : chain_bwd_mt<4, false, false>(P, s);
diff --git a/track_mjx_amd/hip.py b/track_mjx_amd/hip.py
--- a/track_mjx_amd/hip.py
+++ b/track_mjx_amd/hip.py
@@ -81,7 +81,8 @@
 
 class ChainBwd(C.Structure):
     _fields_ = [("G", C.c_void_p), ("ldg", C.c_int32), ("Kg", C.c_int32), ("M", C.c_int32), ("n_stages", C.c_int32), ("epi", C.c_int32), ("stage", ChainBwdStage * 4),
-                ("W0", C.c_void_p), ("ldw0", C.c_int32), ("dx_cols", C.c_int32), ("dx", C.c_void_p), ("lddx", C.c_int32), ("rows_alloc", C.c_int32), ("prof", C.c_void_p)]
+                ("W0", C.c_void_p), ("ldw0", C.c_int32), ("dx_cols", C.c_int32), ("dx", C.c_void_p), ("lddx", C.c_int32), ("rows_alloc", C.c_int32), ("prof", C.c_void_p),
+                ("lat_dx", C.c_void_p), ("lat_eps", C.c_void_p), ("lat_fc2", C.c_void_p), ("lat_add", C.c_void_p), ("lat_Z", C.c_int32), ("lat_ldx", C.c_int32)]
 
 
 class PpoCfg(C.Structure):
```

Result: no change. 1.694 million (median of 6 runs) (-0.0%).
